# HarborYuan/PolyphonicFormer

Hardware: AMD Instinct MI355X
Metric: frames/sec kernel-update+mask fwd, 1024x2048 N=153 S=3 (higher is better)
Workload: dtype bf16 (feature planes as given; query side: updator half hi/lo bf16, attention / FFN / towers one fp16 plane; one fp16 plane of dynamic kernels, fp16 logits)

## Files before the change

### polyphonicformer_amd/csrc/ph_query.hip

```cpp
#include <stdlib.h>

#include "ph_common.h"

template <int E> __device__ __forceinline__ uint32_t q_f2e(float x) {
    if constexpr (E == PH_E_F16) return f2h(__builtin_amdgcn_fmed3f(x, -65504.f, 65504.f));
    else return f2bf(x);
}

constexpr int LDA = 264;
constexpr float LN_EPS = 1e-5f;

constexpr int NW = 8;
constexpr int CT = 2;
constexpr int WCOLS = CT * 16;
constexpr int NTHREADS = NW * 64;

template <int NRT> struct Tile { f32x4_t v[NRT][CT]; };


struct QArgs {
    const float* partial; const uint32_t* bits; const float* k_in; const float* q_in;
    const uint16_t* wb; const float* wf;
    float* obj; float* dobj; float* cls; uint16_t* kern; float* kbias;
    uint16_t* Qp; uint16_t* Kp; uint16_t* Vt; float* o1;
    ph_stage_layout lay;
    int nsplit, B, N, Npad, cls_sigmoid, kern_f16;
    int64_t HWp;
    const int32_t* pcount;
};

__device__ __forceinline__ int q_lane(int lane) {
    asm volatile("" : "+v"(lane));
    return lane;
}

template <int NRT> __device__ __forceinline__ void tile_zero(f32x4_t (&a)[NRT][CT]) {
#pragma unroll
    for (int rt = 0; rt < NRT; ++rt)
#pragma unroll
        for (int ct = 0; ct < CT; ++ct) a[rt][ct] = f32x4_t{0.f, 0.f, 0.f, 0.f};
}

template <int NRT>
__device__ __forceinline__ void tile_add_bias(Tile<NRT>& t, const float* __restrict__ bias, int wave, int lane) {
#pragma unroll
    for (int ct = 0; ct < CT; ++ct) {
        const float bv = bias[wave * WCOLS + ct * 16 + (lane & 15)];
#pragma unroll
        for (int rt = 0; rt < NRT; ++rt)
#pragma unroll
            for (int r = 0; r < 4; ++r) t.v[rt][ct][r] += bv;
    }
}

template <int PA, int NRT, int E = PH_E_BF16>
__device__ __forceinline__ void tile_to_lds(const Tile<NRT>& t, uint16_t* dst, int plane, int wave, int lane) {
    lane = q_lane(lane);
    const int i = lane & 15, g = lane >> 4;
#pragma unroll
    for (int rt = 0; rt < NRT; ++rt)
#pragma unroll
        for (int ct = 0; ct < CT; ++ct)
#pragma unroll
            for (int r = 0; r < 4; ++r) {
                const int off = (rt * 16 + g * 4 + r) * LDA + wave * WCOLS + ct * 16 + i;
                if (PA == 1) dst[off] = (uint16_t)q_f2e<E>(t.v[rt][ct][r]);
                else {
                    uint32_t hi, lo;
                    f2bf_split(t.v[rt][ct][r], hi, lo);
                    dst[off] = (uint16_t)hi;
                    dst[off + plane] = (uint16_t)lo;
                }
            }
}

template <int NRT, int NT>
__device__ __forceinline__ void ln_row_totals(float* red, int pass, int tid) {
    constexpr int ROWS = NRT * 16;
    for (int idx = tid; idx < NT * ROWS; idx += NTHREADS) {
        float* p = red + ((pass * NT + idx / ROWS) * NW) * ROWS + idx % ROWS;
        float tot = 0.f;
#pragma unroll
        for (int w = 0; w < NW; ++w) tot += p[w * ROWS];
        p[0] = tot;
    }
    __syncthreads();
}
template <int NRT, int NT>
__device__ __forceinline__ void ln_tiles(Tile<NRT> (&t)[NT], const float* const (&gam)[NT], const float* const (&bet)[NT],
                                         float* red, int wave, int lane) {
    constexpr int ROWS = NRT * 16;
    lane = q_lane(lane);
    const int i = lane & 15, g = lane >> 4;
    float mean[NT][NRT][4];
#pragma unroll
    for (int n = 0; n < NT; ++n)
#pragma unroll
        for (int rt = 0; rt < NRT; ++rt)
#pragma unroll
            for (int r = 0; r < 4; ++r) {
                float s = 0.f;
#pragma unroll
                for (int ct = 0; ct < CT; ++ct) s += t[n].v[rt][ct][r];
                s = wave_group16_sum(s);
                if (i == 0) red[((0 * NT + n) * NW + wave) * ROWS + rt * 16 + g * 4 + r] = s;
            }
    __syncthreads();
    ln_row_totals<NRT, NT>(red, 0, wave * 64 + lane);
#pragma unroll
    for (int n = 0; n < NT; ++n)
#pragma unroll
        for (int rt = 0; rt < NRT; ++rt) {
            __builtin_amdgcn_sched_barrier(0);
            asm volatile("" ::: "memory");
#pragma unroll
            for (int r = 0; r < 4; ++r) {
                const float tot = red[(0 * NT + n) * NW * ROWS + rt * 16 + g * 4 + r];
                mean[n][rt][r] = tot * (1.f / 256.f);
                float s = 0.f;
#pragma unroll
                for (int ct = 0; ct < CT; ++ct) {
                    const float d = t[n].v[rt][ct][r] - mean[n][rt][r];
                    t[n].v[rt][ct][r] = d;
                    s += d * d;
                }
                s = wave_group16_sum(s);
                if (i == 0) red[((1 * NT + n) * NW + wave) * ROWS + rt * 16 + g * 4 + r] = s;
            }
#pragma unroll
            for (int ct = 0; ct < CT; ++ct) asm volatile("" : "+v"(t[n].v[rt][ct]));
        }
    __syncthreads();
    ln_row_totals<NRT, NT>(red, 1, wave * 64 + lane);
#pragma unroll
    for (int n = 0; n < NT; ++n) {
        float gm[CT], bt[CT];
#pragma unroll
        for (int ct = 0; ct < CT; ++ct) {
            gm[ct] = gam[n][wave * WCOLS + ct * 16 + i];
            bt[ct] = bet[n][wave * WCOLS + ct * 16 + i];
        }
#pragma unroll
        for (int rt = 0; rt < NRT; ++rt) {
            __builtin_amdgcn_sched_barrier(0);
            asm volatile("" ::: "memory");
#pragma unroll
            for (int r = 0; r < 4; ++r) {
                const float tot = red[(1 * NT + n) * NW * ROWS + rt * 16 + g * 4 + r];
                const float var = tot * (1.f / 256.f);
                const float rstd = fast_rsqrt(var + LN_EPS);
#pragma unroll
                for (int ct = 0; ct < CT; ++ct) t[n].v[rt][ct][r] = t[n].v[rt][ct][r] * rstd * gm[ct] + bt[ct];
            }
#pragma unroll
            for (int ct = 0; ct < CT; ++ct) asm volatile("" : "+v"(t[n].v[rt][ct]));
        }
    }
}

template <int PA, int NRT, int PART, bool QF16 = false>
__device__ __forceinline__ void store_qkv(const Tile<NRT>& T, const QArgs& a, const float* bias, int64_t qk_base,
                                          int64_t qk_plane, int64_t vt_base, int wave, int lane) {
    lane = q_lane(lane);
    const int i = lane & 15, g = lane >> 4;
#pragma unroll
    for (int ct = 0; ct < CT; ++ct) {
        const int col = wave * WCOLS + ct * 16 + i;
        const float bv = bias[col];
#pragma unroll
        for (int rt = 0; rt < NRT; ++rt) {
            uint32_t hi[4], lo[4];
#pragma unroll
            for (int r = 0; r < 4; ++r) {
                float v = T.v[rt][ct][r] + bv;
                if (PART == 0) v *= 0.17677669529663687f;
                if (QF16) { hi[r] = q_f2e<PH_E_F16>(v); lo[r] = 0; }
                else if (PA == 2) f2bf_split(v, hi[r], lo[r]);
                else hi[r] = f2bf(v);
            }
            if (PART < 2) {
                uint16_t* dst = (PART == 0 ? a.Qp : a.Kp) + qk_base + (rt * 16 + g * 4) * 256 + col;
#pragma unroll
                for (int r = 0; r < 4; ++r) {
                    dst[r * 256] = (uint16_t)hi[r];
                    if (PA == 2 && !QF16) dst[qk_plane + r * 256] = (uint16_t)lo[r];
                }
            } else {
                uint16_t* dst = a.Vt + vt_base + (int64_t)col * a.Npad + rt * 16 + g * 4;
                *(uint2*)dst = make_uint2(pack2(hi[0], hi[1]), pack2(hi[2], hi[3]));
                if (PA == 2 && !QF16) *(uint2*)(dst + qk_plane) = make_uint2(pack2(lo[0], lo[1]), pack2(lo[2], lo[3]));
            }
        }
    }
}

constexpr int LDPT = 40;

struct WRef2 { const uint16_t* W; int ct0, ks_total, wks0; };
template <int PA> constexpr int kch() { return PA == 1 ? 4 : 2; }
template <int NCT> struct WStreamF { uint4 f[2][4][NCT]; };
template <int PA, int NCT> using WStream = WStreamF<NCT>;

template <int PA, int NCT>
__device__ __forceinline__ void w_chunk_load(uint4 (&d)[4][NCT], const WRef2& r, int kc, int64_t w_plane, int lane) {
#pragma unroll
    for (int p = 0; p < PA; ++p)
#pragma unroll
        for (int k = 0; k < kch<PA>(); ++k)
#pragma unroll
            for (int ct = 0; ct < NCT; ++ct)
                d[p * kch<PA>() + k][ct] = *(const uint4*)(r.W + p * w_plane + ((int64_t)(r.ct0 + ct) * r.ks_total + r.wks0 + kc * kch<PA>() + k) * 512 + lane * 8);
}
template <int PA, int NCT>
__device__ __forceinline__ void w_prime(WStream<PA, NCT>& ws, const WRef2& r, int64_t w_plane, int lane) {
    w_chunk_load<PA, NCT>(ws.f[0], r, 0, w_plane, lane);
}
struct NoNext { __device__ __forceinline__ void operator()() const {} };

template <int PA, int NRT, int NCT, int NKS, int E = PH_E_BF16, typename Next>
__device__ __forceinline__ void gemm_stream(f32x4_t (&acc)[NRT][NCT], const uint16_t* A, int lda, int a_plane, WStream<PA, NCT>& ws,
                                            const WRef2& r, int64_t w_plane, int lane, Next next) {
    constexpr int KCH = kch<PA>(), NCH = NKS / KCH;
    static_assert(NKS % KCH == 0 && NCH % 2 == 0, "a call is an even number of chunks");
    constexpr int RG = PA == 2 ? 1 : (NRT < 2 ? NRT : 2);
    const int i = lane & 15, g = lane >> 4;
    __builtin_amdgcn_sched_barrier(0);
#pragma unroll
    for (int kc = 0; kc < NCH; ++kc) {
        if (kc + 1 < NCH) w_chunk_load<PA, NCT>(ws.f[(kc + 1) & 1], r, kc + 1, w_plane, lane);
        else next();
        __builtin_amdgcn_sched_barrier(0);
#pragma unroll
        for (int k = 0; k < KCH; ++k)
#pragma unroll
            for (int rt0 = 0; rt0 < NRT; rt0 += RG) {
                uint4 a[PA][RG];
#pragma unroll
                for (int p = 0; p < PA; ++p)
#pragma unroll
                    for (int rr = 0; rr < RG && rt0 + rr < NRT; ++rr)
                        a[p][rr] = *(const uint4*)(A + p * a_plane + ((rt0 + rr) * 16 + i) * lda + (kc * KCH + k) * 32 + g * 8);
#pragma unroll
                for (int ct = 0; ct < NCT; ++ct)
#pragma unroll
                    for (int rr = 0; rr < RG && rt0 + rr < NRT; ++rr) {
                        f32x4_t& c = acc[rt0 + rr][ct];
                        c = mfma16e<E>(a[0][rr], ws.f[kc & 1][k][ct], c);
                        if (PA == 2) {
                            c = mfma16(a[0][rr], ws.f[kc & 1][(PA - 1) * KCH + k][ct], c);
                            c = mfma16(a[PA - 1][rr], ws.f[kc & 1][k][ct], c);
                        }
                    }
            }
        __builtin_amdgcn_sched_barrier(0);
    }
}

template <int PA, int NRT, int NCT, int E = PH_E_BF16>
__device__ __forceinline__ void frag_to_lds(const f32x4_t (&t)[NRT][NCT], uint16_t* dst, int ld, int plane, int col0, int lane) {
    lane = q_lane(lane);
    const int i = lane & 15, g = lane >> 4;
#pragma unroll
    for (int rt = 0; rt < NRT; ++rt)
#pragma unroll
        for (int ct = 0; ct < NCT; ++ct)
#pragma unroll
            for (int r = 0; r < 4; ++r) {
                const int off = (rt * 16 + g * 4 + r) * ld + col0 + ct * 16 + i;
                if (PA == 1) dst[off] = (uint16_t)q_f2e<E>(t[rt][ct][r]);
                else {
                    uint32_t hi, lo;
                    f2bf_split(t[rt][ct][r], hi, lo);
                    dst[off] = (uint16_t)hi;
                    dst[off + plane] = (uint16_t)lo;
                }
            }
}

struct QArgs2 {
    QArgs q;
    unsigned long long* tl;
    float* pi;
    int br0, nbr;
};

#define PH_TL(k)                                                                                             \
    do {                                                                                                     \
        if (aa.tl && blockIdx.x == 0 && blockIdx.y == 0 && blockIdx.z == 0 && threadIdx.x == 0)              \
            aa.tl[(k)] = __builtin_amdgcn_s_memrealtime();                                                   \
    } while (0)

template <int PA, int NRT, bool QF16 = false>
__global__ __launch_bounds__(NTHREADS) void k_query_pre2(const QArgs2 aa) {
    const QArgs& a = aa.q;
    constexpr int ROWS = NRT * 16;
    constexpr int PLANE = ROWS * LDA;
    extern __shared__ __attribute__((aligned(16))) unsigned char smem[];
    uint16_t* act = (uint16_t*)smem;
    float* red = (float*)(act + PA * PLANE);
    float* cnt = red + 2 * 2 * NW * ROWS;

    const int tid = threadIdx.x, lane = tid & 63;
    const int wave = __builtin_amdgcn_readfirstlane(tid >> 6);
    const int i = lane & 15, g = lane >> 4;
    const int row0 = blockIdx.x * ROWS, br = blockIdx.y + aa.br0, b = blockIdx.z;
    const int N = a.N, Npad = a.Npad;
    const uint16_t* wb = a.wb;
    const int64_t wpl = a.lay.wb_plane_elems;
    const float* wf = a.wf;
    const int64_t* WO = a.lay.w[br];
    const int64_t* VO = a.lay.v[br];
    float* pi = aa.pi + ((((int64_t)b * 2 + br) * Npad + row0) * 2) * 256;

    WStream<PA, CT> ws;
    const WRef2 c_dyn_o{wb + WO[PH_W_DYN], 16 + wave * CT, 8, 0}, c_dyn_i{wb + WO[PH_W_DYN], wave * CT, 8, 0};
    const WRef2 c_inp_i{wb + WO[PH_W_INP], wave * CT, 8, 0}, c_inp_o{wb + WO[PH_W_INP], 16 + wave * CT, 8, 0};
    const WRef2 c_ug{wb + WO[PH_W_UG], wave * CT, 8, 0}, c_ig{wb + WO[PH_W_IG], wave * CT, 8, 0}, c_fc{wb + WO[PH_W_FC], wave * CT, 8, 0};
    const WRef2 c_q{wb + WO[PH_W_QKV], wave * CT, 8, 0}, c_k{wb + WO[PH_W_QKV], 16 + wave * CT, 8, 0}, c_v{wb + WO[PH_W_QKV], 32 + wave * CT, 8, 0};
    auto prime = [&](const WRef2& r) { return [&, r]() { w_prime<PA, CT>(ws, r, wpl, lane); }; };
    constexpr int PT = QF16 ? 1 : PA;
    constexpr int ET = QF16 ? PH_E_F16 : PH_E_BF16;
    auto primeT = [&](const WRef2& r) { return [&, r]() { w_prime<PT, CT>(ws, r, wpl, lane); }; };
    w_prime<PA, CT>(ws, c_dyn_o, wpl, lane);
    PH_TL(0);

    auto put16 = [&](int rr, int cb, const float (&v)[16]) {
#pragma unroll
        for (int e = 0; e < 16; e += 2) {
            uint32_t h0, l0, h1, l1;
            f2bf_split(v[e], h0, l0); f2bf_split(v[e + 1], h1, l1);
            *(uint32_t*)(act + rr * LDA + cb + e) = pack2(h0, h1);
            if (PA == 2) *(uint32_t*)(act + PLANE + rr * LDA + cb + e) = pack2(l0, l1);
        }
    };

    {
        const int r = tid >> 5, cb = (tid & 31) * 8;
        for (int rr = r; rr < ROWS; rr += NTHREADS / 32) {
            const int row = row0 + rr;
            float u[8];
#pragma unroll
            for (int e = 0; e < 8; ++e) u[e] = 0.f;
            int c = 0;
            if (row < Npad) {
                if (a.pcount) {
                    for (int s0 = tid & 31; s0 < a.nsplit; s0 += 32) c += a.pcount[((int64_t)b * a.nsplit + s0) * Npad + row];
                } else {
                    const uint4* bw = (const uint4*)(a.bits + ((int64_t)b * Npad + row) * (a.HWp / 32));
                    const int nq = (int)(a.HWp / 128);
                    for (int w0 = tid & 31; w0 < nq; w0 += 256) {
                        uint4 q[8];
#pragma unroll
                        for (int j = 0; j < 8; ++j) q[j] = w0 + 32 * j < nq ? bw[w0 + 32 * j] : make_uint4(0, 0, 0, 0);
#pragma unroll
                        for (int j = 0; j < 8; ++j) c += __popc(q[j].x) + __popc(q[j].y) + __popc(q[j].z) + __popc(q[j].w);
                    }
                }
                constexpr int TRIP = NRT == 1 ? 16 : 8;
                for (int s0 = 0; s0 < a.nsplit; s0 += TRIP) {
                    float4 v[TRIP][2];
#pragma unroll
                    for (int j = 0; j < TRIP; ++j) {
                        const float* p = a.partial + (((int64_t)b * a.nsplit + s0 + j) * Npad + row) * 512 + br * 256 + cb;
#pragma unroll
                        for (int e = 0; e < 2; ++e)
                            v[j][e] = s0 + j < a.nsplit ? *(const float4*)(p + 4 * e) : make_float4(0.f, 0.f, 0.f, 0.f);
                    }
#pragma unroll
                    for (int j = 0; j < TRIP; ++j)
#pragma unroll
                        for (int e = 0; e < 2; ++e) {
                            u[4 * e] += v[j][e].x; u[4 * e + 1] += v[j][e].y; u[4 * e + 2] += v[j][e].z; u[4 * e + 3] += v[j][e].w;
                        }
                }
            }
#pragma unroll
            for (int e = 0; e < 8; e += 2) {
                uint32_t h0, l0, h1, l1;
                f2bf_split(u[e], h0, l0); f2bf_split(u[e + 1], h1, l1);
                *(uint32_t*)(act + rr * LDA + cb + e) = pack2(h0, h1);
                if (PA == 2) *(uint32_t*)(act + PLANE + rr * LDA + cb + e) = pack2(l0, l1);
            }
            float cf = wave_group16_sum((float)c);
            cf += __shfl_xor(cf, 16);
            if ((tid & 31) == 0) cnt[rr] = cf;
        }
    }
    __syncthreads();

    PH_TL(1);
    const float* vc = wf + VO[PH_V_DYN_CNT];
    const float* bd = wf + VO[PH_V_DYN_B];
    {
        Tile<NRT> Po[1];
        tile_zero(Po[0].v);
        const int lp = q_lane(lane), i = lp & 15, g = lp >> 4;
        gemm_stream<PA, NRT, CT, 8>(Po[0].v, act, LDA, PLANE, ws, c_dyn_o, wpl, lane, prime(c_dyn_i));
#pragma unroll
        for (int ct = 0; ct < CT; ++ct) {
            const int col = wave * WCOLS + ct * 16 + i;
            const float vc1 = vc[256 + col], bd1 = bd[256 + col];
#pragma unroll
            for (int rt = 0; rt < NRT; ++rt)
#pragma unroll
                for (int r = 0; r < 4; ++r) Po[0].v[rt][ct][r] += cnt[rt * 16 + g * 4 + r] * vc1 + bd1;
        }
        const float* const gm[1] = {wf + VO[PH_V_LN_PO_G]};
        const float* const bt[1] = {wf + VO[PH_V_LN_PO_B]};
        ln_tiles<NRT, 1>(Po, gm, bt, red, wave, lane);
#pragma unroll
        for (int rt = 0; rt < NRT; ++rt)
#pragma unroll
            for (int ct = 0; ct < CT; ++ct)
#pragma unroll
                for (int r = 0; r < 4; ++r)
                    pi[((rt * 16 + g * 4 + r) * 2 + 0) * 256 + wave * WCOLS + ct * 16 + i] = Po[0].v[rt][ct][r];
    }
    Tile<NRT> Pin;
    tile_zero(Pin.v);
    gemm_stream<PA, NRT, CT, 8>(Pin.v, act, LDA, PLANE, ws, c_dyn_i, wpl, lane, prime(c_inp_i));
    {
        const int lp = q_lane(lane), i = lp & 15, g = lp >> 4;
#pragma unroll
        for (int ct = 0; ct < CT; ++ct) {
            const int col = wave * WCOLS + ct * 16 + i;
            const float vc0 = vc[col], bd0 = bd[col];
#pragma unroll
            for (int rt = 0; rt < NRT; ++rt)
#pragma unroll
                for (int r = 0; r < 4; ++r) Pin.v[rt][ct][r] += cnt[rt * 16 + g * 4 + r] * vc0 + bd0;
        }
    }
    __syncthreads();
    PH_TL(2);
    {
        const int r = tid >> 4, cb = (tid & 15) * 16;
        for (int rr = r; rr < ROWS; rr += NTHREADS / 16) {
            const int row = row0 + rr;
            float kv[16];
#pragma unroll
            for (int e = 0; e < 16; ++e) kv[e] = 0.f;
            if (row < N) {
                const float* kp = a.k_in + ((int64_t)b * N + row) * 256 + cb;
#pragma unroll
                for (int e = 0; e < 16; e += 4) {
                    const float4 v = *(const float4*)(kp + e);
                    kv[e] = v.x; kv[e + 1] = v.y; kv[e + 2] = v.z; kv[e + 3] = v.w;
                }
                if (br == 1) {
                    const float* qp = a.q_in + ((int64_t)b * N + row) * 256 + cb;
#pragma unroll
                    for (int e = 0; e < 16; e += 4) {
                        const float4 v = *(const float4*)(qp + e);
                        kv[e] += v.x; kv[e + 1] += v.y; kv[e + 2] += v.z; kv[e + 3] += v.w;
                    }
                }
            }
            put16(rr, cb, kv);
        }
    }
    __syncthreads();
    PH_TL(3);
    const float* bi = wf + VO[PH_V_INP_B];
    {
        Tile<NRT> Iin;
        tile_zero(Iin.v);
        const int lp = q_lane(lane), i = lp & 15, g = lp >> 4;
        gemm_stream<PA, NRT, CT, 8>(Iin.v, act, LDA, PLANE, ws, c_inp_i, wpl, lane, prime(c_inp_o));
#pragma unroll
        for (int ct = 0; ct < CT; ++ct) {
            const float bi0 = bi[wave * WCOLS + ct * 16 + i];
#pragma unroll
            for (int rt = 0; rt < NRT; ++rt)
#pragma unroll
                for (int r = 0; r < 4; ++r) Pin.v[rt][ct][r] = (Iin.v[rt][ct][r] + bi0) * Pin.v[rt][ct][r];
        }
    }
    {
        Tile<NRT> Io[1];
        tile_zero(Io[0].v);
        const int lp = q_lane(lane), i = lp & 15, g = lp >> 4;
        gemm_stream<PA, NRT, CT, 8>(Io[0].v, act, LDA, PLANE, ws, c_inp_o, wpl, lane, prime(c_ug));
#pragma unroll
        for (int ct = 0; ct < CT; ++ct) {
            const float bi1 = bi[256 + wave * WCOLS + ct * 16 + i];
#pragma unroll
            for (int rt = 0; rt < NRT; ++rt)
#pragma unroll
                for (int r = 0; r < 4; ++r) Io[0].v[rt][ct][r] += bi1;
        }
        const float* const gm[1] = {wf + VO[PH_V_LN_IO_G]};
        const float* const bt[1] = {wf + VO[PH_V_LN_IO_B]};
        ln_tiles<NRT, 1>(Io, gm, bt, red, wave, lane);
#pragma unroll
        for (int rt = 0; rt < NRT; ++rt)
#pragma unroll
            for (int ct = 0; ct < CT; ++ct)
#pragma unroll
                for (int r = 0; r < 4; ++r)
                    pi[((rt * 16 + g * 4 + r) * 2 + 1) * 256 + wave * WCOLS + ct * 16 + i] = Io[0].v[rt][ct][r];
    }
    tile_to_lds<PA, NRT>(Pin, act, PLANE, wave, lane);
    __syncthreads();

    PH_TL(4);
    {
        Tile<NRT> Fg;
        auto gate = [&](const WRef2& cur, auto&& next, int b_idx, int g_idx, int be_idx, int which, bool first) {
            Tile<NRT> G[1];
            tile_zero(G[0].v);
            gemm_stream<PA, NRT, CT, 8>(G[0].v, act, LDA, PLANE, ws, cur, wpl, lane, next);
            tile_add_bias(G[0], wf + VO[b_idx], wave, lane);
            const float* const gm[1] = {wf + VO[g_idx]};
            const float* const bt[1] = {wf + VO[be_idx]};
            ln_tiles<NRT, 1>(G, gm, bt, red, wave, lane);
            const int lp = q_lane(lane), i = lp & 15, g = lp >> 4;
#pragma unroll
            for (int rt = 0; rt < NRT; ++rt) {
                float pv[CT][4];
#pragma unroll
                for (int ct = 0; ct < CT; ++ct)
#pragma unroll
                    for (int r = 0; r < 4; ++r) pv[ct][r] = pi[((rt * 16 + g * 4 + r) * 2 + which) * 256 + wave * WCOLS + ct * 16 + i];
#pragma unroll
                for (int ct = 0; ct < CT; ++ct)
#pragma unroll
                    for (int r = 0; r < 4; ++r) {
                        const float t = fast_sigmoid(G[0].v[rt][ct][r]) * pv[ct][r];
                        Fg.v[rt][ct][r] = first ? t : Fg.v[rt][ct][r] + t;
                    }
            }
        };
        gate(c_ug, prime(c_ig), PH_V_UG_B, PH_V_LN_UG_G, PH_V_LN_UG_B, 0, true);
        gate(c_ig, prime(c_fc), PH_V_IG_B, PH_V_LN_IG_G, PH_V_LN_IG_B, 1, false);
        tile_to_lds<PA, NRT>(Fg, act, PLANE, wave, lane);
    }
    __syncthreads();

    PH_TL(5);
    {
        Tile<NRT> O[1];
        tile_zero(O[0].v);
        gemm_stream<PA, NRT, CT, 8>(O[0].v, act, LDA, PLANE, ws, c_fc, wpl, lane, primeT(c_q));
        tile_add_bias(O[0], wf + VO[PH_V_FC_B], wave, lane);
        const float* const gm[1] = {wf + VO[PH_V_LN_FC_G]};
        const float* const bt[1] = {wf + VO[PH_V_LN_FC_B]};
        ln_tiles<NRT, 1>(O, gm, bt, red, wave, lane);
        const int lp = q_lane(lane), i = lp & 15, g = lp >> 4;
        float* o1 = a.o1 + (((int64_t)b * 2 + br) * Npad + row0) * 256;
#pragma unroll
        for (int rt = 0; rt < NRT; ++rt)
#pragma unroll
            for (int ct = 0; ct < CT; ++ct)
#pragma unroll
                for (int r = 0; r < 4; ++r) {
                    const float v = fmaxf(O[0].v[rt][ct][r], 0.f);
                    O[0].v[rt][ct][r] = v;
                    o1[(rt * 16 + g * 4 + r) * 256 + wave * WCOLS + ct * 16 + i] = v;
                }
        tile_to_lds<PT, NRT, ET>(O[0], act, PLANE, wave, lane);
    }
    __syncthreads();

    PH_TL(6);
    const int64_t qk_base = (((int64_t)b * 2 + br) * Npad + row0) * 256;
    const int64_t qk_plane = (int64_t)a.B * 2 * Npad * 256;
    const int64_t vt_base = ((int64_t)b * 2 + br) * 256 * Npad + row0;
    const float* qkv_bias = wf + VO[PH_V_QKV_B];
    {
        Tile<NRT> T;
        tile_zero(T.v);
        gemm_stream<PT, NRT, CT, 8, ET>(T.v, act, LDA, PLANE, ws, c_q, wpl, lane, primeT(c_k));
        store_qkv<PA, NRT, 0, QF16>(T, a, qkv_bias, qk_base, qk_plane, vt_base, wave, lane);
        tile_zero(T.v);
        gemm_stream<PT, NRT, CT, 8, ET>(T.v, act, LDA, PLANE, ws, c_k, wpl, lane, primeT(c_v));
        store_qkv<PA, NRT, 1, QF16>(T, a, qkv_bias + 256, qk_base, qk_plane, vt_base, wave, lane);
        tile_zero(T.v);
        gemm_stream<PT, NRT, CT, 8, ET>(T.v, act, LDA, PLANE, ws, c_v, wpl, lane, NoNext());
        store_qkv<PA, NRT, 2, QF16>(T, a, qkv_bias + 512, qk_base, qk_plane, vt_base, wave, lane);
    }
    PH_TL(7);
}

template <int PA> constexpr int post2_hc() { return PA == 1 ? 256 : 128; }
template <int PA, int NRT> constexpr int post2_nhb() {
    return ((size_t)PA * NRT * 16 * LDA * 2 + 2 * (size_t)PA * NRT * 16 * (post2_hc<PA>() + 8) * 2 + 2 * 2 * NW * NRT * 16 * 4 + NW * PA * 16 * LDPT * 2 <= 150 * 1024) ? 2 : 1;
}

template <int PA, int NRT, int E = PH_E_BF16>
__global__ __launch_bounds__(NTHREADS) void k_query_post2(const QArgs2 aa) {
    const QArgs& a = aa.q;
    constexpr int ROWS = NRT * 16;
    constexpr int PLANE = ROWS * LDA;
    constexpr int HC = post2_hc<PA>(), LDH = HC + 8, CTH = HC / 128;
    constexpr int HPLANE = ROWS * LDH;
    constexpr int NHB = post2_nhb<PA, NRT>();
    extern __shared__ __attribute__((aligned(16))) unsigned char smem[];
    uint16_t* act = (uint16_t*)smem;
    uint16_t* hb = act + PA * PLANE;
    float* red = (float*)(hb + NHB * PA * HPLANE);
    uint16_t* ptile = (uint16_t*)(red + 2 * 2 * NW * ROWS);
    const int Npad = a.Npad, N = a.N;

    const int tid = threadIdx.x, lane = tid & 63;
    const int wave = __builtin_amdgcn_readfirstlane(tid >> 6);
    const int i = lane & 15, g = lane >> 4;
    const int row0 = blockIdx.x * ROWS, br = blockIdx.y + aa.br0, b = blockIdx.z;
    const uint16_t* wb = a.wb;
    const int64_t wpl = a.lay.wb_plane_elems;
    const float* wf = a.wf;
    const int64_t* WO = a.lay.w[br];
    const int64_t* VO = a.lay.v[br];

    const int64_t qk_plane = (int64_t)a.B * 2 * Npad * 256;
    const uint16_t* Qb = a.Qp + (((int64_t)b * 2 + br) * Npad + row0) * 256;
    const uint16_t* Kb = a.Kp + ((int64_t)b * 2 + br) * Npad * 256;
    const uint16_t* Vb = a.Vt + ((int64_t)b * 2 + br) * 256 * Npad;

    WStream<PA, CT> ws;
    WStream<PA, 1> ws1;
    const WRef2 c_out{wb + WO[PH_W_OUT], wave * CT, 8, 0};
    const WRef2 c_h0a{wb + WO[PH_W_H0A], wave * CT, 8, 0}, c_h0b{wb + WO[PH_W_H0B], wave * CT, 8, 0};
    const WRef2 c_kern{wb + WO[PH_W_KERN], wave * CT, 8, 0}, c_kb{wb + WO[PH_W_KERN], 16, 8, 0};
    auto prime = [&](const WRef2& r) { return [&, r]() { w_prime<PA, CT>(ws, r, wpl, lane); }; };
    auto ffn1_ref = [&](int c) { return WRef2{wb + WO[PH_W_FFN1], c * (HC / 16) + wave * CTH, 8, 0}; };
    auto ffn1_prime = [&](int c) {
        if constexpr (CTH == CT) w_prime<PA, CT>(ws, ffn1_ref(c), wpl, lane);
        else w_prime<PA, 1>(ws1, ffn1_ref(c), wpl, lane);
    };
    w_prime<PA, CT>(ws, c_out, wpl, lane);
    PH_TL(8);

    Tile<NRT> At;
    {
        const int h = wave;
        const int nkt = Npad / 16;
        uint16_t* Pt = ptile + wave * (PA * 16 * LDPT);
        uint4 qf[PA][NRT];
#pragma unroll
        for (int p = 0; p < PA; ++p)
#pragma unroll
            for (int rt = 0; rt < NRT; ++rt)
                qf[p][rt] = *(const uint4*)(Qb + p * qk_plane + (rt * 16 + i) * 256 + h * 32 + g * 8);
        float mx[NRT][4], sm[NRT][4];
#pragma unroll
        for (int rt = 0; rt < NRT; ++rt)
#pragma unroll
            for (int r = 0; r < 4; ++r) { mx[rt][r] = -INFINITY; sm[rt][r] = 0.f; }
        auto load_k = [&](uint4 (&kf)[PA], int kt) {
#pragma unroll
            for (int p = 0; p < PA; ++p) kf[p] = *(const uint4*)(Kb + p * qk_plane + (kt * 16 + i) * 256 + h * 32 + g * 8);
        };
        auto score = [&](const uint4 (&kf)[PA], int rt) {
            f32x4_t s = {0.f, 0.f, 0.f, 0.f};
            s = mfma16e<E>(qf[0][rt], kf[0], s);
            if (PA == 2) { s = mfma16(qf[0][rt], kf[PA - 1], s); s = mfma16(qf[PA - 1][rt], kf[0], s); }
            return s;
        };
        for (int kt = 0; kt < nkt; ++kt) {
            uint4 kf[PA];
            load_k(kf, kt);
            const bool valid = kt * 16 + i < N;
#pragma unroll
            for (int rt = 0; rt < NRT; ++rt) {
                const f32x4_t s = score(kf, rt);
#pragma unroll
                for (int r = 0; r < 4; ++r) mx[rt][r] = fmaxf(mx[rt][r], valid ? s[r] : -INFINITY);
            }
        }
#pragma unroll
        for (int rt = 0; rt < NRT; ++rt)
#pragma unroll
            for (int r = 0; r < 4; ++r) mx[rt][r] = wave_group16_max(mx[rt][r]);
        tile_zero(At.v);
        for (int ks = 0; ks < nkt / 2; ++ks) {
            uint4 kf[2][PA], vf[2][PA];
            load_k(kf[0], 2 * ks);
            load_k(kf[1], 2 * ks + 1);
#pragma unroll
            for (int ct = 0; ct < 2; ++ct)
#pragma unroll
                for (int p = 0; p < PA; ++p)
                    vf[ct][p] = *(const uint4*)(Vb + p * qk_plane + (int64_t)(h * 32 + ct * 16 + i) * Npad + ks * 32 + g * 8);
#pragma unroll
            for (int rt = 0; rt < NRT; ++rt) {
#pragma unroll
                for (int half = 0; half < 2; ++half) {
                    const f32x4_t s = score(kf[half], rt);
                    const bool valid = (2 * ks + half) * 16 + i < N;
#pragma unroll
                    for (int r = 0; r < 4; ++r) {
                        const float pv = valid ? fast_exp(s[r] - mx[rt][r]) : 0.f;
                        sm[rt][r] += pv;
                        const int off = (g * 4 + r) * LDPT + half * 16 + i;
                        if (PA == 2) {
                            uint32_t hi, lo;
                            f2bf_split(pv, hi, lo);
                            Pt[off] = (uint16_t)hi;
                            Pt[16 * LDPT + off] = (uint16_t)lo;
                        } else Pt[off] = (uint16_t)q_f2e<E>(pv);
                    }
                }
                uint4 pf[PA];
#pragma unroll
                for (int p = 0; p < PA; ++p) pf[p] = *(const uint4*)(Pt + p * 16 * LDPT + i * LDPT + g * 8);
#pragma unroll
                for (int ct = 0; ct < 2; ++ct) {
                    At.v[rt][ct] = mfma16e<E>(pf[0], vf[ct][0], At.v[rt][ct]);
                    if (PA == 2) {
                        At.v[rt][ct] = mfma16(pf[0], vf[ct][PA - 1], At.v[rt][ct]);
                        At.v[rt][ct] = mfma16(pf[PA - 1], vf[ct][0], At.v[rt][ct]);
                    }
                }
            }
        }
#pragma unroll
        for (int rt = 0; rt < NRT; ++rt)
#pragma unroll
            for (int r = 0; r < 4; ++r) {
                const float inv = fast_rcp(wave_group16_sum(sm[rt][r]));
#pragma unroll
                for (int ct = 0; ct < 2; ++ct) At.v[rt][ct][r] *= inv;
            }
    }
    tile_to_lds<PA, NRT, E>(At, act, PLANE, wave, lane);
    __syncthreads();

    PH_TL(9);
    Tile<NRT> O2[1];
    tile_zero(O2[0].v);
    gemm_stream<PA, NRT, CT, 8, E>(O2[0].v, act, LDA, PLANE, ws, c_out, wpl, lane, [&]() { ffn1_prime(0); });
    tile_add_bias(O2[0], wf + VO[PH_V_OUT_B], wave, lane);
    {
        const float* o1 = a.o1 + (((int64_t)b * 2 + br) * Npad + row0) * 256;
#pragma unroll
        for (int rt = 0; rt < NRT; ++rt)
#pragma unroll
            for (int ct = 0; ct < CT; ++ct)
#pragma unroll
                for (int r = 0; r < 4; ++r) O2[0].v[rt][ct][r] += o1[(rt * 16 + g * 4 + r) * 256 + wave * WCOLS + ct * 16 + i];
        const float* const gm[1] = {wf + VO[PH_V_LN_ATT_G]};
        const float* const bt[1] = {wf + VO[PH_V_LN_ATT_B]};
        ln_tiles<NRT, 1>(O2, gm, bt, red, wave, lane);
    }
    tile_to_lds<PA, NRT, E>(O2[0], act, PLANE, wave, lane);
    float* park = aa.pi + ((((int64_t)b * 2 + br) * Npad + row0) * 2) * 256;
#pragma unroll
    for (int rt = 0; rt < NRT; ++rt)
#pragma unroll
        for (int ct = 0; ct < CT; ++ct)
#pragma unroll
            for (int r = 0; r < 4; ++r) park[(rt * 16 + g * 4 + r) * 512 + wave * WCOLS + ct * 16 + i] = O2[0].v[rt][ct][r];
    __syncthreads();

    PH_TL(10);
    Tile<NRT> O3[1];
    tile_zero(O3[0].v);
    {
        const int nchunk = a.lay.ffn_dim / HC;
        const int ffn_ks = a.lay.ffn_dim / 32;
        for (int c = 0; c < nchunk; ++c) {
            uint16_t* hc = hb + (NHB == 2 ? (c & 1) : 0) * PA * HPLANE;
            const WRef2 w2{wb + WO[PH_W_FFN2], wave * CT, ffn_ks, c * (HC / 32)};
            f32x4_t Hc[NRT][CTH];
#pragma unroll
            for (int rt = 0; rt < NRT; ++rt)
#pragma unroll
                for (int ct = 0; ct < CTH; ++ct) Hc[rt][ct] = f32x4_t{0.f, 0.f, 0.f, 0.f};
            if constexpr (CTH == CT) gemm_stream<PA, NRT, CT, 8, E>(Hc, act, LDA, PLANE, ws, ffn1_ref(c), wpl, lane, prime(w2));
            else gemm_stream<PA, NRT, 1, 8, E>(Hc, act, LDA, PLANE, ws1, ffn1_ref(c), wpl, lane, prime(w2));
#pragma unroll
            for (int ct = 0; ct < CTH; ++ct) {
                const float bv = (wf + VO[PH_V_FFN1_B])[c * HC + (wave * CTH + ct) * 16 + i];
#pragma unroll
                for (int rt = 0; rt < NRT; ++rt)
#pragma unroll
                    for (int r = 0; r < 4; ++r) Hc[rt][ct][r] = fmaxf(Hc[rt][ct][r] + bv, 0.f);
            }
            if (NHB == 1 && c > 0) __syncthreads();
            frag_to_lds<PA, NRT, CTH, E>(Hc, hc, LDH, HPLANE, wave * CTH * 16, lane);
            __syncthreads();
            gemm_stream<PA, NRT, CT, HC / 32, E>(O3[0].v, hc, LDH, HPLANE, ws, w2, wpl, lane, [&]() {
                if (c + 1 < nchunk) ffn1_prime(c + 1);
                else w_prime<PA, CT>(ws, br == 0 ? c_h0b : c_h0a, wpl, lane);
            });
        }
    }
    PH_TL(11);
    tile_add_bias(O3[0], wf + VO[PH_V_FFN2_B], wave, lane);
#pragma unroll
    for (int rt = 0; rt < NRT; ++rt)
#pragma unroll
        for (int ct = 0; ct < CT; ++ct)
#pragma unroll
            for (int r = 0; r < 4; ++r) O3[0].v[rt][ct][r] += park[(rt * 16 + g * 4 + r) * 512 + wave * WCOLS + ct * 16 + i];
    {
        const float* const gm[1] = {wf + VO[PH_V_LN_FFN_G]};
        const float* const bt[1] = {wf + VO[PH_V_LN_FFN_B]};
        ln_tiles<NRT, 1>(O3, gm, bt, red, wave, lane);
    }
    {
        float* out = (br == 0 ? a.obj : a.dobj) + ((int64_t)b * N + row0) * 256;
#pragma unroll
        for (int rt = 0; rt < NRT; ++rt)
#pragma unroll
            for (int ct = 0; ct < CT; ++ct)
#pragma unroll
                for (int r = 0; r < 4; ++r) {
                    const int rr = rt * 16 + g * 4 + r;
                    if (row0 + rr < N) out[rr * 256 + wave * WCOLS + ct * 16 + i] = O3[0].v[rt][ct][r];
                }
    }
    tile_to_lds<PA, NRT, E>(O3[0], act, PLANE, wave, lane);
    __syncthreads();

    PH_TL(12);
    Tile<NRT> Hm[1];
    if (br == 0) {
        tile_zero(Hm[0].v);
        gemm_stream<PA, NRT, CT, 8, E>(Hm[0].v, act, LDA, PLANE, ws, c_h0b, wpl, lane, prime(c_h0a));
        {
            const float* const gm[1] = {wf + VO[PH_V_LN_H0B_G]};
            const float* const bt[1] = {wf + VO[PH_V_LN_H0B_B]};
            ln_tiles<NRT, 1>(Hm, gm, bt, red, wave, lane);
        }
        Tile<NRT> Hd[1];
        tile_zero(Hd[0].v);
        const int L = a.lay.num_classes, nct = (L + 15) / 16;
        auto cls_ref = [&](int ct) { return WRef2{wb + WO[PH_W_CLS], ct, 8, 0}; };
        gemm_stream<PA, NRT, CT, 8, E>(Hd[0].v, act, LDA, PLANE, ws, c_h0a, wpl, lane, [&]() {
            w_prime<PA, CT>(ws, c_kern, wpl, lane);
            if (wave < nct) w_prime<PA, 1>(ws1, cls_ref(wave), wpl, lane);
        });
        {
            const float* const gm[1] = {wf + VO[PH_V_LN_H0A_G]};
            const float* const bt[1] = {wf + VO[PH_V_LN_H0A_B]};
            ln_tiles<NRT, 1>(Hd, gm, bt, red, wave, lane);
        }
#pragma unroll
        for (int rt = 0; rt < NRT; ++rt)
#pragma unroll
            for (int ct = 0; ct < CT; ++ct)
#pragma unroll
                for (int r = 0; r < 4; ++r) {
                    Hd[0].v[rt][ct][r] = fmaxf(Hd[0].v[rt][ct][r], 0.f);
                    Hm[0].v[rt][ct][r] = fmaxf(Hm[0].v[rt][ct][r], 0.f);
                }
        tile_to_lds<PA, NRT, E>(Hd[0], act, PLANE, wave, lane);
        __syncthreads();
        const float* bc = wf + VO[PH_V_CLS_B];
        for (int ct = wave; ct < nct; ct += NW) {
            f32x4_t acc[NRT][1];
#pragma unroll
            for (int rt = 0; rt < NRT; ++rt) acc[rt][0] = f32x4_t{0.f, 0.f, 0.f, 0.f};
            gemm_stream<PA, NRT, 1, 8, E>(acc, act, LDA, PLANE, ws1, cls_ref(ct), wpl, lane, [&]() {
                if (ct + NW < nct) w_prime<PA, 1>(ws1, cls_ref(ct + NW), wpl, lane);
            });
            const int col = ct * 16 + i;
            if (col < L) {
                const float bv = bc[col];
#pragma unroll
                for (int rt = 0; rt < NRT; ++rt)
#pragma unroll
                    for (int r = 0; r < 4; ++r) {
                        const int row = row0 + rt * 16 + g * 4 + r;
                        if (row < N) {
                            const float z = acc[rt][0][r] + bv;
                            a.cls[((int64_t)b * N + row) * L + col] = a.cls_sigmoid ? fast_sigmoid(z) : z;
                        }
                    }
            }
        }
        __syncthreads();
    } else {
        tile_zero(Hm[0].v);
        gemm_stream<PA, NRT, CT, 8, E>(Hm[0].v, act, LDA, PLANE, ws, c_h0a, wpl, lane, prime(c_kern));
        const float* const gm[1] = {wf + VO[PH_V_LN_H0A_G]};
        const float* const bt[1] = {wf + VO[PH_V_LN_H0A_B]};
        ln_tiles<NRT, 1>(Hm, gm, bt, red, wave, lane);
    }
    tile_to_lds<PA, NRT, E>(Hm[0], act, PLANE, wave, lane);
    __syncthreads();
    {
        Tile<NRT> Kt;
        tile_zero(Kt.v);
        gemm_stream<PA, NRT, CT, 8, E>(Kt.v, act, LDA, PLANE, ws, c_kern, wpl, lane, [&]() {
            if (wave == 0) w_prime<PA, 1>(ws1, c_kb, wpl, lane);
        });
        const float* bk = wf + VO[PH_V_KERN_B];
        const int64_t kplane = (int64_t)2 * a.B * Npad * 256;
        uint16_t* kd = a.kern + (((int64_t)br * a.B + b) * Npad + row0) * 256;
#pragma unroll
        for (int ct = 0; ct < CT; ++ct) {
            const int col = wave * WCOLS + ct * 16 + i;
            const float bv = bk[col];
#pragma unroll
            for (int rt = 0; rt < NRT; ++rt)
#pragma unroll
                for (int r = 0; r < 4; ++r) {
                    const int off = (rt * 16 + g * 4 + r) * 256 + col;
                    if (a.kern_f16) {
                        kd[off] = (uint16_t)q_f2e<PH_E_F16>(Kt.v[rt][ct][r] + bv);
                    } else {
                        uint32_t hi, lo;
                        f2bf_split(Kt.v[rt][ct][r] + bv, hi, lo);
                        kd[off] = (uint16_t)hi;
                        if (PA == 2) kd[kplane + off] = (uint16_t)lo;
                    }
                }
        }
        if (wave == 0) {
            f32x4_t acc[NRT][1];
#pragma unroll
            for (int rt = 0; rt < NRT; ++rt) acc[rt][0] = f32x4_t{0.f, 0.f, 0.f, 0.f};
            gemm_stream<PA, NRT, 1, 8, E>(acc, act, LDA, PLANE, ws1, c_kb, wpl, lane, NoNext());
            if (i == 0) {
                const float bv = bk[256];
#pragma unroll
                for (int rt = 0; rt < NRT; ++rt)
#pragma unroll
                    for (int r = 0; r < 4; ++r)
                        a.kbias[((int64_t)br * a.B + b) * Npad + row0 + rt * 16 + g * 4 + r] = acc[rt][0][r] + bv;
            }
        }
    }
    PH_TL(13);
}

static size_t q_ws_bytes(int B, int Npad, int PA) {
    return (size_t)PA * 3 * B * 2 * Npad * 256 * sizeof(uint16_t) + (size_t)3 * B * 2 * Npad * 256 * sizeof(float);
}

extern "C" size_t ph_query_workspace_updator_offset(int B, int N, int prec) {
    return (size_t)((prec == PH_PREC_SPLIT || prec == PH_PREC_QHYBRID) ? 2 : 1) * 3 * B * 2 * ph_n_padded(N) * 256 * sizeof(uint16_t);
}

extern "C" size_t ph_query_workspace_bytes(int B, int N, int prec) {
    return q_ws_bytes(B, ph_n_padded(N), (prec == PH_PREC_SPLIT || prec == PH_PREC_QHYBRID) ? 2 : 1);
}

template <int PA, int NRT, bool HY = false>
static void launch_query2(const QArgs2& a, int phases, hipStream_t s) {
    constexpr int ROWS = NRT * 16;
    if constexpr (HY) {
        static_assert(PA == 2, "hybrid = split pre kernel");
        const size_t red = 2 * 2 * NW * ROWS * sizeof(float);
        const size_t lds_pre = (size_t)2 * ROWS * LDA * 2 + red + ROWS * sizeof(float);
        const size_t lds_post = (size_t)ROWS * LDA * 2 + (size_t)post2_nhb<1, NRT>() * ROWS * (post2_hc<1>() + 8) * 2 + red + (size_t)NW * 16 * LDPT * 2;
        static const bool once = [] {
            (void)hipFuncSetAttribute((const void*)k_query_pre2<2, NRT, true>, hipFuncAttributeMaxDynamicSharedMemorySize, 160 * 1024);
            (void)hipFuncSetAttribute((const void*)k_query_post2<1, NRT, PH_E_F16>, hipFuncAttributeMaxDynamicSharedMemorySize, 160 * 1024);
            return true;
        }();
        (void)once;
        const dim3 grid(a.q.Npad / ROWS, a.nbr, a.q.B);
        if (phases & 1) hipLaunchKernelGGL((k_query_pre2<2, NRT, true>), grid, dim3(NTHREADS), lds_pre, s, a);
        if (phases & 2) hipLaunchKernelGGL((k_query_post2<1, NRT, PH_E_F16>), grid, dim3(NTHREADS), lds_post, s, a);
        return;
    }
    const size_t red = 2 * 2 * NW * ROWS * sizeof(float);
    const size_t lds_pre = (size_t)PA * ROWS * LDA * 2 + red + ROWS * sizeof(float);
    const size_t lds_post = (size_t)PA * ROWS * LDA * 2 + (size_t)post2_nhb<PA, NRT>() * PA * ROWS * (post2_hc<PA>() + 8) * 2 + red +
                            (size_t)NW * PA * 16 * LDPT * 2;
    static const bool once = [] {
        (void)hipFuncSetAttribute((const void*)k_query_pre2<PA, NRT>, hipFuncAttributeMaxDynamicSharedMemorySize, 160 * 1024);
        (void)hipFuncSetAttribute((const void*)k_query_post2<PA, NRT>, hipFuncAttributeMaxDynamicSharedMemorySize, 160 * 1024);
        return true;
    }();
    (void)once;
    const dim3 grid(a.q.Npad / ROWS, a.nbr, a.q.B);
    if (phases & 1) hipLaunchKernelGGL((k_query_pre2<PA, NRT>), grid, dim3(NTHREADS), lds_pre, s, a);
    if (phases & 2) hipLaunchKernelGGL((k_query_post2<PA, NRT>), grid, dim3(NTHREADS), lds_post, s, a);
}

static int query_run(const PhQueryKnobs& kn, const float* partial, int nsplit, const uint32_t* bits, const int32_t* pcount, const float* k_in,
                     const float* q_in, const uint16_t* wb, const float* wf, const ph_stage_layout* layout, float* obj, float* dobj,
                     float* cls, int cls_sigmoid, uint16_t* kern, float* kbias, void* workspace,
                     size_t workspace_bytes, int B, int N, int64_t HW, int prec, int kern_format, int phases,
                     void* stream) {
    PH_CHECK_ARG((phases & ~(PH_QUERY_BOTH | PH_QUERY_WIDE | PH_QUERY_MASK_ONLY | PH_QUERY_DEPTH_ONLY)) == 0 && (phases & PH_QUERY_BOTH) != 0 &&
                     (phases & (PH_QUERY_MASK_ONLY | PH_QUERY_DEPTH_ONLY)) != (PH_QUERY_MASK_ONLY | PH_QUERY_DEPTH_ONLY),
                 "phases must be PH_QUERY_PRE | PH_QUERY_POST [| PH_QUERY_WIDE] [| PH_QUERY_MASK_ONLY or PH_QUERY_DEPTH_ONLY]");
    PH_CHECK_ARG(partial && bits && k_in && q_in && wb && wf && layout && obj && dobj && cls && kern && kbias && workspace,
                 "null pointer");
    PH_CHECK_ARG(B > 0 && N > 0 && N <= 256 && HW > 0 && nsplit >= 1, "bad size");
    PH_CHECK_ARG(prec == PH_PREC_BF16 || prec == PH_PREC_SPLIT || prec == PH_PREC_QHYBRID, "prec must be PH_PREC_BF16, PH_PREC_SPLIT or PH_PREC_QHYBRID");
    PH_CHECK_ARG(kern_format == PH_KERN_BF16_PLANES || kern_format == PH_KERN_F16, "bad kern_format");
    PH_CHECK_ARG(prec != PH_PREC_QHYBRID || kern_format == PH_KERN_F16, "PH_PREC_QHYBRID emits the dynamic kernels as one fp16 plane (PH_KERN_F16)");
    PH_CHECK_ARG(layout->ffn_dim > 0 && layout->ffn_dim % 256 == 0, "ffn_dim must be a multiple of 256");
    PH_CHECK_ARG(layout->num_classes > 0 && layout->num_classes <= 1024, "bad num_classes");
    const bool hybrid = prec == PH_PREC_QHYBRID;
    const int PA = (prec == PH_PREC_SPLIT || hybrid) ? 2 : 1, Npad = ph_n_padded(N);
    const bool wide = (phases & PH_QUERY_WIDE) != 0;
    const int br0 = (phases & PH_QUERY_DEPTH_ONLY) ? 1 : 0, nbr = (phases & (PH_QUERY_MASK_ONLY | PH_QUERY_DEPTH_ONLY)) ? 1 : 2;
    phases &= PH_QUERY_BOTH;
    if (workspace_bytes < q_ws_bytes(B, Npad, PA)) {
        ph_set_error("ph_query_stage: workspace too small (%zu < %zu)", workspace_bytes, q_ws_bytes(B, Npad, PA));
        return PH_EWORKSPACE;
    }
    QArgs a;
    a.partial = partial; a.bits = bits; a.pcount = pcount; a.k_in = k_in; a.q_in = q_in; a.wb = wb; a.wf = wf;
    a.obj = obj; a.dobj = dobj; a.cls = cls; a.kern = kern; a.kbias = kbias;
    const size_t pl = (size_t)PA * B * 2 * Npad * 256;
    a.Qp = (uint16_t*)workspace; a.Kp = a.Qp + pl; a.Vt = a.Kp + pl; a.o1 = (float*)(a.Vt + pl);
    a.lay = *layout; a.cls_sigmoid = cls_sigmoid; a.kern_f16 = kern_format == PH_KERN_F16; a.nsplit = nsplit; a.B = B; a.N = N; a.Npad = Npad; a.HWp = ph_hw_padded(HW);
    hipStream_t s = (hipStream_t)stream;
    QArgs2 a2;
    a2.q = a;
    unsigned long long* tl = kn.timeline;
    a2.tl = tl;
    a2.pi = a.o1 + (size_t)B * 2 * Npad * 256;
    a2.br0 = br0; a2.nbr = nbr;
    const int t = Npad / 16;
    int nrt = 1;
    if (wide) {
        nrt = t % 5 == 0 ? 5 : (t % 4 == 0 ? 4 : (t % 3 == 0 ? 3 : (t % 2 == 0 ? 2 : 1)));
    } else {
        int smallest = 1;
        for (int c = 5; c >= 2; --c) {
            if (t % c) continue;
            smallest = c;
            if (nrt == 1 && (int64_t)B * 2 * (t / c) >= 200) nrt = c;
        }
        if (nrt == 1) nrt = smallest;
    }
    if (kn.nrt > 0) { nrt = kn.nrt; while (t % nrt) --nrt; }
#define PH_Q2(P, R) launch_query2<P, R>(a2, phases, s)
#define PH_QH(R) launch_query2<2, R, true>(a2, phases, s)
    if (hybrid) { switch (nrt) { case 5: PH_QH(5); break; case 4: PH_QH(4); break; case 3: PH_QH(3); break; case 2: PH_QH(2); break; default: PH_QH(1); } }
    else if (PA == 1) { switch (nrt) { case 5: PH_Q2(1, 5); break; case 4: PH_Q2(1, 4); break; case 3: PH_Q2(1, 3); break; case 2: PH_Q2(1, 2); break; default: PH_Q2(1, 1); } }
    else { switch (nrt) { case 5: PH_Q2(2, 5); break; case 4: PH_Q2(2, 4); break; case 3: PH_Q2(2, 3); break; case 2: PH_Q2(2, 2); break; default: PH_Q2(2, 1); } }
#undef PH_Q2
#undef PH_QH
    if (tl) {
        unsigned long long h[16];
        (void)hipStreamSynchronize(s);
        (void)hipMemcpy(h, tl, sizeof(h), hipMemcpyDeviceToHost);
        fprintf(stderr, "query timeline (100 MHz ticks, x10 ns):");
        for (int k = 1; k < 14; ++k) fprintf(stderr, " %s%lld", k == 8 ? "| " : "", (long long)(h[k] - h[k - 1]));
        fprintf(stderr, "\n");
    }
    PH_CHECK_LAUNCH();
    return PH_OK;
}

static PhQueryKnobs query_switches() {
    PhQueryKnobs k;
    k.nrt = ph_switch(PH_SWITCH_QUERY_NRT);
    if (ph_switch(PH_SWITCH_QUERY_TIMELINE)) {
        static unsigned long long* const tl = [] {
            unsigned long long* p = nullptr;
            if (hipMalloc((void**)&p, 16 * sizeof(unsigned long long)) == hipSuccess) (void)hipMemset(p, 0, 128);
            return p;
        }();
        k.timeline = tl;
    }
    return k;
}

extern "C" int ph_query_stage(const float* partial, int nsplit, const uint32_t* bits, const float* k_in, const float* q_in,
                              const uint16_t* wb, const float* wf, const ph_stage_layout* layout, float* obj, float* dobj,
                              float* cls, int cls_sigmoid, uint16_t* kern, float* kbias, void* workspace,
                              size_t workspace_bytes, int B, int N, int64_t HW, int prec, int kern_format, int phases,
                              void* stream) {
    return query_run(query_switches(), partial, nsplit, bits, nullptr, k_in, q_in, wb, wf, layout, obj, dobj, cls, cls_sigmoid, kern, kbias, workspace,
                     workspace_bytes, B, N, HW, prec, kern_format, phases, stream);
}

extern "C" int ph_query_stage_counts(const float* partial, int nsplit, const uint32_t* bits, const int32_t* pcount, const float* k_in,
                                     const float* q_in, const uint16_t* wb, const float* wf, const ph_stage_layout* layout,
                                     float* obj, float* dobj, float* cls, int cls_sigmoid, uint16_t* kern, float* kbias,
                                     void* workspace, size_t workspace_bytes, int B, int N, int64_t HW, int prec, int kern_format,
                                     int phases, void* stream) {
    if (!pcount) { ph_set_error("ph_query_stage_counts: null pcount"); return PH_EINVAL; }
    return query_run(query_switches(), partial, nsplit, bits, pcount, k_in, q_in, wb, wf, layout, obj, dobj, cls, cls_sigmoid, kern, kbias,
                     workspace, workspace_bytes, B, N, HW, prec, kern_format, phases, stream);
}

int ph_query_stage_counts_k(const PhQueryKnobs& kn, const float* partial, int nsplit, const uint32_t* bits, const int32_t* pcount,
                            const float* k_in, const float* q_in, const uint16_t* wb, const float* wf, const ph_stage_layout* layout,
                            float* obj, float* dobj, float* cls, int cls_sigmoid, uint16_t* kern, float* kbias, void* workspace,
                            size_t workspace_bytes, int B, int N, int64_t HW, int prec, int kern_format, int phases, void* stream) {
    if (!pcount) { ph_set_error("ph_query_stage_counts: null pcount"); return PH_EINVAL; }
    return query_run(kn, partial, nsplit, bits, pcount, k_in, q_in, wb, wf, layout, obj, dobj, cls, cls_sigmoid, kern, kbias, workspace,
                     workspace_bytes, B, N, HW, prec, kern_format, phases, stream);
}
```

Before: 18150.

## Swap MFMA operands so query-side accumulators hold rows per lane, vectorize epilogues

Adds a RowLane fragment layout in which gemm_stream swaps the MFMA A/B operands. Each lane then holds four consecutive columns of one row instead of four rows of one column. LayerNorm row reductions, bias adds, LDS writebacks and the global stores of Q/K, dynamic kernels and class logits can then use 4-wide vector accesses and cheaper two-step shuffles, in place of scalar 16-bit stores and 16-lane group sums. V^T keeps the old column layout. This touches many epilogues at once, and the new vector paths rely on alignment assumptions, with a scalar fallback kept for cls.

Result: no change. 18060 (-0.5%).

```diff
diff --git a/polyphonicformer_amd/csrc/ph_query.hip b/polyphonicformer_amd/csrc/ph_query.hip
--- a/polyphonicformer_amd/csrc/ph_query.hip
+++ b/polyphonicformer_amd/csrc/ph_query.hip
@@ -15,7 +15,10 @@
 constexpr int WCOLS = CT * 16;
 constexpr int NTHREADS = NW * 64;
 
-template <int NRT> struct Tile { f32x4_t v[NRT][CT]; };
+struct RowLane {};
+struct ColLane {};
+template <int NRT, int NCT, typename LAY = RowLane> struct Frag { f32x4_t v[NRT][NCT]; };
+template <int NRT, typename LAY = RowLane> using Tile = Frag<NRT, CT, LAY>;
 
 
 struct QArgs {
@@ -34,36 +37,68 @@
     return lane;
 }
 
-template <int NRT> __device__ __forceinline__ void tile_zero(f32x4_t (&a)[NRT][CT]) {
+__device__ __forceinline__ int q_uniform(int x) {
+    asm volatile("" : "+s"(x));
+    return x;
+}
+
+template <int NRT, int NCT, typename LAY> __device__ __forceinline__ void tile_zero(Frag<NRT, NCT, LAY>& t) {
 #pragma unroll
     for (int rt = 0; rt < NRT; ++rt)
 #pragma unroll
-        for (int ct = 0; ct < CT; ++ct) a[rt][ct] = f32x4_t{0.f, 0.f, 0.f, 0.f};
-}
-
-template <int NRT>
-__device__ __forceinline__ void tile_add_bias(Tile<NRT>& t, const float* __restrict__ bias, int wave, int lane) {
-#pragma unroll
-    for (int ct = 0; ct < CT; ++ct) {
-        const float bv = bias[wave * WCOLS + ct * 16 + (lane & 15)];
-#pragma unroll
-        for (int rt = 0; rt < NRT; ++rt)
-#pragma unroll
-            for (int r = 0; r < 4; ++r) t.v[rt][ct][r] += bv;
-    }
-}
-
-template <int PA, int NRT, int E = PH_E_BF16>
-__device__ __forceinline__ void tile_to_lds(const Tile<NRT>& t, uint16_t* dst, int plane, int wave, int lane) {
+        for (int ct = 0; ct < NCT; ++ct) t.v[rt][ct] = f32x4_t{0.f, 0.f, 0.f, 0.f};
+}
+
+__device__ __forceinline__ f32x4_t ld4(const float* p) { return *(const f32x4_t*)p; }
+__device__ __forceinline__ void st4(float* p, f32x4_t v) { *(f32x4_t*)p = v; }
+
+template <int PA, int E>
+__device__ __forceinline__ void pack4(f32x4_t v, uint2& hi, uint2& lo) {
+    uint32_t h[4], l[4];
+#pragma unroll
+    for (int r = 0; r < 4; ++r) {
+        if (PA == 1) { h[r] = q_f2e<E>(v[r]); l[r] = 0; }
+        else f2bf_split(v[r], h[r], l[r]);
+    }
+    hi = make_uint2(pack2(h[0], h[1]), pack2(h[2], h[3]));
+    lo = make_uint2(pack2(l[0], l[1]), pack2(l[2], l[3]));
+}
+
+template <int NRT, int NCT>
+__device__ __forceinline__ void tile_add_bias(Frag<NRT, NCT, RowLane>& t, const float* __restrict__ bias, int lane) {
+#pragma unroll
+    for (int ct = 0; ct < NCT; ++ct) {
+        const f32x4_t bv = ld4(bias + ct * 16 + (lane >> 4) * 4);
+#pragma unroll
+        for (int rt = 0; rt < NRT; ++rt) t.v[rt][ct] += bv;
+    }
+}
+
+template <int PA, int E = PH_E_BF16, int NRT, int NCT>
+__device__ __forceinline__ void frag_to_lds(const Frag<NRT, NCT, RowLane>& t, uint16_t* dst, int ld, int plane, int col0, int lane) {
+    lane = q_lane(lane);
+    uint16_t* d = dst + (lane & 15) * ld + col0 + (lane >> 4) * 4;
+#pragma unroll
+    for (int rt = 0; rt < NRT; ++rt)
+#pragma unroll
+        for (int ct = 0; ct < NCT; ++ct) {
+            uint2 hi, lo;
+            pack4<PA, E>(t.v[rt][ct], hi, lo);
+            *(uint2*)(d + rt * 16 * ld + ct * 16) = hi;
+            if (PA == 2) *(uint2*)(d + plane + rt * 16 * ld + ct * 16) = lo;
+        }
+}
+template <int PA, int E = PH_E_BF16, int NRT, int NCT>
+__device__ __forceinline__ void frag_to_lds(const Frag<NRT, NCT, ColLane>& t, uint16_t* dst, int ld, int plane, int col0, int lane) {
     lane = q_lane(lane);
     const int i = lane & 15, g = lane >> 4;
 #pragma unroll
     for (int rt = 0; rt < NRT; ++rt)
 #pragma unroll
-        for (int ct = 0; ct < CT; ++ct)
+        for (int ct = 0; ct < NCT; ++ct)
 #pragma unroll
             for (int r = 0; r < 4; ++r) {
-                const int off = (rt * 16 + g * 4 + r) * LDA + wave * WCOLS + ct * 16 + i;
+                const int off = (rt * 16 + g * 4 + r) * ld + col0 + ct * 16 + i;
                 if (PA == 1) dst[off] = (uint16_t)q_f2e<E>(t.v[rt][ct][r]);
                 else {
                     uint32_t hi, lo;
@@ -73,6 +108,10 @@
                 }
             }
 }
+template <int PA, int NRT, int E = PH_E_BF16, typename LAY>
+__device__ __forceinline__ void tile_to_lds(const Tile<NRT, LAY>& t, uint16_t* dst, int plane, int wave, int lane) {
+    frag_to_lds<PA, E>(t, dst, LDA, plane, wave * WCOLS, lane);
+}
 
 template <int NRT, int NT>
 __device__ __forceinline__ void ln_row_totals(float* red, int pass, int tid) {
@@ -86,81 +125,97 @@
     }
     __syncthreads();
 }
+__device__ __forceinline__ float row4_sum(float s) {
+    s += __shfl_xor(s, 16);
+    s += __shfl_xor(s, 32);
+    return s;
+}
 template <int NRT, int NT>
-__device__ __forceinline__ void ln_tiles(Tile<NRT> (&t)[NT], const float* const (&gam)[NT], const float* const (&bet)[NT],
+__device__ __forceinline__ void ln_tiles(Tile<NRT, RowLane> (&t)[NT], const float* const (&gam)[NT], const float* const (&bet)[NT],
                                          float* red, int wave, int lane) {
     constexpr int ROWS = NRT * 16;
+    const int i = lane & 15, g = lane >> 4;
+#pragma unroll
+    for (int n = 0; n < NT; ++n)
+#pragma unroll
+        for (int rt = 0; rt < NRT; ++rt) {
+            float p[4];
+#pragma unroll
+            for (int r = 0; r < 4; ++r) {
+                p[r] = 0.f;
+#pragma unroll
+                for (int ct = 0; ct < CT; ++ct) p[r] += t[n].v[rt][ct][r];
+            }
+            const float s = row4_sum((p[0] + p[1]) + (p[2] + p[3]));
+            if (g == 0) red[((0 * NT + n) * NW + wave) * ROWS + rt * 16 + i] = s;
+        }
+    __syncthreads();
+    ln_row_totals<NRT, NT>(red, 0, wave * 64 + lane);
+#pragma unroll
+    for (int n = 0; n < NT; ++n)
+#pragma unroll
+        for (int rt = 0; rt < NRT; ++rt) {
+            const float mean = red[(0 * NT + n) * NW * ROWS + rt * 16 + i] * (1.f / 256.f);
+            float p[4];
+#pragma unroll
+            for (int r = 0; r < 4; ++r) {
+                p[r] = 0.f;
+#pragma unroll
+                for (int ct = 0; ct < CT; ++ct) {
+                    const float d = t[n].v[rt][ct][r] - mean;
+                    t[n].v[rt][ct][r] = d;
+                    p[r] += d * d;
+                }
+            }
+            const float s = row4_sum((p[0] + p[1]) + (p[2] + p[3]));
+            if (g == 0) red[((1 * NT + n) * NW + wave) * ROWS + rt * 16 + i] = s;
+        }
+    __syncthreads();
+    ln_row_totals<NRT, NT>(red, 1, wave * 64 + lane);
+#pragma unroll
+    for (int n = 0; n < NT; ++n) {
+        f32x4_t gm[CT], bt[CT];
+#pragma unroll
+        for (int ct = 0; ct < CT; ++ct) {
+            gm[ct] = ld4(gam[n] + wave * WCOLS + ct * 16 + g * 4);
+            bt[ct] = ld4(bet[n] + wave * WCOLS + ct * 16 + g * 4);
+        }
+#pragma unroll
+        for (int rt = 0; rt < NRT; ++rt) {
+            const float var = red[(1 * NT + n) * NW * ROWS + rt * 16 + i] * (1.f / 256.f);
+            const float rstd = fast_rsqrt(var + LN_EPS);
+#pragma unroll
+            for (int ct = 0; ct < CT; ++ct) t[n].v[rt][ct] = t[n].v[rt][ct] * rstd * gm[ct] + bt[ct];
+        }
+    }
+}
+
+template <int PA, int NRT, int PART, bool QF16 = false>
+__device__ __forceinline__ void store_qkv(const Tile<NRT, RowLane>& T, const QArgs& a, const float* bias, int64_t qk_base,
+                                          int64_t qk_plane, int64_t vt_base, int wave, int lane) {
+    static_assert(PART < 2, "V^T is stored from a ColLane tile");
+    constexpr int PS = QF16 ? 1 : PA, ES = QF16 ? PH_E_F16 : PH_E_BF16;
     lane = q_lane(lane);
-    const int i = lane & 15, g = lane >> 4;
-    float mean[NT][NRT][4];
-#pragma unroll
-    for (int n = 0; n < NT; ++n)
-#pragma unroll
-        for (int rt = 0; rt < NRT; ++rt)
-#pragma unroll
-            for (int r = 0; r < 4; ++r) {
-                float s = 0.f;
-#pragma unroll
-                for (int ct = 0; ct < CT; ++ct) s += t[n].v[rt][ct][r];
-                s = wave_group16_sum(s);
-                if (i == 0) red[((0 * NT + n) * NW + wave) * ROWS + rt * 16 + g * 4 + r] = s;
-            }
-    __syncthreads();
-    ln_row_totals<NRT, NT>(red, 0, wave * 64 + lane);
-#pragma unroll
-    for (int n = 0; n < NT; ++n)
+    const int col0 = wave * WCOLS + (lane >> 4) * 4;
+    uint16_t* dst = (PART == 0 ? a.Qp : a.Kp) + qk_base + (lane & 15) * 256 + col0;
+#pragma unroll
+    for (int ct = 0; ct < CT; ++ct) {
+        const f32x4_t bv = ld4(bias + col0 + ct * 16);
 #pragma unroll
         for (int rt = 0; rt < NRT; ++rt) {
-            __builtin_amdgcn_sched_barrier(0);
-            asm volatile("" ::: "memory");
-#pragma unroll
-            for (int r = 0; r < 4; ++r) {
-                const float tot = red[(0 * NT + n) * NW * ROWS + rt * 16 + g * 4 + r];
-                mean[n][rt][r] = tot * (1.f / 256.f);
-                float s = 0.f;
-#pragma unroll
-                for (int ct = 0; ct < CT; ++ct) {
-                    const float d = t[n].v[rt][ct][r] - mean[n][rt][r];
-                    t[n].v[rt][ct][r] = d;
-                    s += d * d;
-                }
-                s = wave_group16_sum(s);
-                if (i == 0) red[((1 * NT + n) * NW + wave) * ROWS + rt * 16 + g * 4 + r] = s;
-            }
-#pragma unroll
-            for (int ct = 0; ct < CT; ++ct) asm volatile("" : "+v"(t[n].v[rt][ct]));
-        }
-    __syncthreads();
-    ln_row_totals<NRT, NT>(red, 1, wave * 64 + lane);
-#pragma unroll
-    for (int n = 0; n < NT; ++n) {
-        float gm[CT], bt[CT];
-#pragma unroll
-        for (int ct = 0; ct < CT; ++ct) {
-            gm[ct] = gam[n][wave * WCOLS + ct * 16 + i];
-            bt[ct] = bet[n][wave * WCOLS + ct * 16 + i];
-        }
-#pragma unroll
-        for (int rt = 0; rt < NRT; ++rt) {
-            __builtin_amdgcn_sched_barrier(0);
-            asm volatile("" ::: "memory");
-#pragma unroll
-            for (int r = 0; r < 4; ++r) {
-                const float tot = red[(1 * NT + n) * NW * ROWS + rt * 16 + g * 4 + r];
-                const float var = tot * (1.f / 256.f);
-                const float rstd = fast_rsqrt(var + LN_EPS);
-#pragma unroll
-                for (int ct = 0; ct < CT; ++ct) t[n].v[rt][ct][r] = t[n].v[rt][ct][r] * rstd * gm[ct] + bt[ct];
-            }
-#pragma unroll
-            for (int ct = 0; ct < CT; ++ct) asm volatile("" : "+v"(t[n].v[rt][ct]));
-        }
-    }
-}
-
+            f32x4_t v = T.v[rt][ct] + bv;
+            if (PART == 0) v *= 0.17677669529663687f;
+            uint2 hi, lo;
+            pack4<PS, ES>(v, hi, lo);
+            *(uint2*)(dst + rt * 16 * 256 + ct * 16) = hi;
+            if (PS == 2) *(uint2*)(dst + qk_plane + rt * 16 * 256 + ct * 16) = lo;
+        }
+    }
+}
 template <int PA, int NRT, int PART, bool QF16 = false>
-__device__ __forceinline__ void store_qkv(const Tile<NRT>& T, const QArgs& a, const float* bias, int64_t qk_base,
+__device__ __forceinline__ void store_qkv(const Tile<NRT, ColLane>& T, const QArgs& a, const float* bias, int64_t qk_base,
                                           int64_t qk_plane, int64_t vt_base, int wave, int lane) {
+    static_assert(PART == 2, "Q and K are stored from RowLane tiles");
     lane = q_lane(lane);
     const int i = lane & 15, g = lane >> 4;
 #pragma unroll
@@ -172,24 +227,14 @@
             uint32_t hi[4], lo[4];
 #pragma unroll
             for (int r = 0; r < 4; ++r) {
-                float v = T.v[rt][ct][r] + bv;
-                if (PART == 0) v *= 0.17677669529663687f;
+                const float v = T.v[rt][ct][r] + bv;
                 if (QF16) { hi[r] = q_f2e<PH_E_F16>(v); lo[r] = 0; }
                 else if (PA == 2) f2bf_split(v, hi[r], lo[r]);
                 else hi[r] = f2bf(v);
             }
-            if (PART < 2) {
-                uint16_t* dst = (PART == 0 ? a.Qp : a.Kp) + qk_base + (rt * 16 + g * 4) * 256 + col;
-#pragma unroll
-                for (int r = 0; r < 4; ++r) {
-                    dst[r * 256] = (uint16_t)hi[r];
-                    if (PA == 2 && !QF16) dst[qk_plane + r * 256] = (uint16_t)lo[r];
-                }
-            } else {
-                uint16_t* dst = a.Vt + vt_base + (int64_t)col * a.Npad + rt * 16 + g * 4;
-                *(uint2*)dst = make_uint2(pack2(hi[0], hi[1]), pack2(hi[2], hi[3]));
-                if (PA == 2 && !QF16) *(uint2*)(dst + qk_plane) = make_uint2(pack2(lo[0], lo[1]), pack2(lo[2], lo[3]));
-            }
+            uint16_t* dst = a.Vt + vt_base + (int64_t)col * a.Npad + rt * 16 + g * 4;
+            *(uint2*)dst = make_uint2(pack2(hi[0], hi[1]), pack2(hi[2], hi[3]));
+            if (PA == 2 && !QF16) *(uint2*)(dst + qk_plane) = make_uint2(pack2(lo[0], lo[1]), pack2(lo[2], lo[3]));
         }
     }
 }
@@ -217,9 +262,11 @@
 }
 struct NoNext { __device__ __forceinline__ void operator()() const {} };
 
-template <int PA, int NRT, int NCT, int NKS, int E = PH_E_BF16, typename Next>
-__device__ __forceinline__ void gemm_stream(f32x4_t (&acc)[NRT][NCT], const uint16_t* A, int lda, int a_plane, WStream<PA, NCT>& ws,
+template <int PA, int NKS, int E = PH_E_BF16, int NRT, int NCT, typename LAY, typename Next>
+__device__ __forceinline__ void gemm_stream(Frag<NRT, NCT, LAY>& tile, const uint16_t* A, int lda, int a_plane, WStream<PA, NCT>& ws,
                                             const WRef2& r, int64_t w_plane, int lane, Next next) {
+    constexpr bool SW = __is_same(LAY, RowLane);
+    f32x4_t (&acc)[NRT][NCT] = tile.v;
     constexpr int KCH = kch<PA>(), NCH = NKS / KCH;
     static_assert(NKS % KCH == 0 && NCH % 2 == 0, "a call is an even number of chunks");
     constexpr int RG = PA == 2 ? 1 : (NRT < 2 ? NRT : 2);
@@ -245,36 +292,16 @@
 #pragma unroll
                     for (int rr = 0; rr < RG && rt0 + rr < NRT; ++rr) {
                         f32x4_t& c = acc[rt0 + rr][ct];
-                        c = mfma16e<E>(a[0][rr], ws.f[kc & 1][k][ct], c);
+                        const uint4 &whi = ws.f[kc & 1][k][ct], &wlo = ws.f[kc & 1][(PA - 1) * KCH + k][ct];
+                        c = SW ? mfma16e<E>(whi, a[0][rr], c) : mfma16e<E>(a[0][rr], whi, c);
                         if (PA == 2) {
-                            c = mfma16(a[0][rr], ws.f[kc & 1][(PA - 1) * KCH + k][ct], c);
-                            c = mfma16(a[PA - 1][rr], ws.f[kc & 1][k][ct], c);
+                            c = SW ? mfma16(wlo, a[0][rr], c) : mfma16(a[0][rr], wlo, c);
+                            c = SW ? mfma16(whi, a[PA - 1][rr], c) : mfma16(a[PA - 1][rr], whi, c);
                         }
                     }
             }
         __builtin_amdgcn_sched_barrier(0);
     }
-}
-
-template <int PA, int NRT, int NCT, int E = PH_E_BF16>
-__device__ __forceinline__ void frag_to_lds(const f32x4_t (&t)[NRT][NCT], uint16_t* dst, int ld, int plane, int col0, int lane) {
-    lane = q_lane(lane);
-    const int i = lane & 15, g = lane >> 4;
-#pragma unroll
-    for (int rt = 0; rt < NRT; ++rt)
-#pragma unroll
-        for (int ct = 0; ct < NCT; ++ct)
-#pragma unroll
-            for (int r = 0; r < 4; ++r) {
-                const int off = (rt * 16 + g * 4 + r) * ld + col0 + ct * 16 + i;
-                if (PA == 1) dst[off] = (uint16_t)q_f2e<E>(t[rt][ct][r]);
-                else {
-                    uint32_t hi, lo;
-                    f2bf_split(t[rt][ct][r], hi, lo);
-                    dst[off] = (uint16_t)hi;
-                    dst[off + plane] = (uint16_t)lo;
-                }
-            }
 }
 
 struct QArgs2 {
@@ -303,13 +330,13 @@
     const int tid = threadIdx.x, lane = tid & 63;
     const int wave = __builtin_amdgcn_readfirstlane(tid >> 6);
     const int i = lane & 15, g = lane >> 4;
+    const int col0 = wave * WCOLS + g * 4;
     const int row0 = blockIdx.x * ROWS, br = blockIdx.y + aa.br0, b = blockIdx.z;
     const int N = a.N, Npad = a.Npad;
     const uint16_t* wb = a.wb;
     const int64_t wpl = a.lay.wb_plane_elems;
     const float* wf = a.wf;
     const int64_t* WO = a.lay.w[br];
-    const int64_t* VO = a.lay.v[br];
     float* pi = aa.pi + ((((int64_t)b * 2 + br) * Npad + row0) * 2) * 256;
 
     WStream<PA, CT> ws;
@@ -318,6 +345,14 @@
     const WRef2 c_ug{wb + WO[PH_W_UG], wave * CT, 8, 0}, c_ig{wb + WO[PH_W_IG], wave * CT, 8, 0}, c_fc{wb + WO[PH_W_FC], wave * CT, 8, 0};
     const WRef2 c_q{wb + WO[PH_W_QKV], wave * CT, 8, 0}, c_k{wb + WO[PH_W_QKV], 16 + wave * CT, 8, 0}, c_v{wb + WO[PH_W_QKV], 32 + wave * CT, 8, 0};
     auto prime = [&](const WRef2& r) { return [&, r]() { w_prime<PA, CT>(ws, r, wpl, lane); }; };
+    auto park_store = [&](const Tile<NRT>& t, float* dst, int ld) {
+        const int lp = q_lane(lane);
+        float* d = dst + (lp & 15) * ld + wave * WCOLS + (lp >> 4) * 4;
+#pragma unroll
+        for (int rt = 0; rt < NRT; ++rt)
+#pragma unroll
+            for (int ct = 0; ct < CT; ++ct) st4(d + rt * 16 * ld + ct * 16, t.v[rt][ct]);
+    };
     constexpr int PT = QF16 ? 1 : PA;
     constexpr int ET = QF16 ? PH_E_F16 : PH_E_BF16;
     auto primeT = [&](const WRef2& r) { return [&, r]() { w_prime<PT, CT>(ws, r, wpl, lane); }; };
@@ -389,48 +424,33 @@
     __syncthreads();
 
     PH_TL(1);
-    const float* vc = wf + VO[PH_V_DYN_CNT];
-    const float* bd = wf + VO[PH_V_DYN_B];
+    const float* vc = wf + a.lay.v[q_uniform(br)][PH_V_DYN_CNT];
+    const float* bd = wf + a.lay.v[q_uniform(br)][PH_V_DYN_B];
+    auto add_cnt = [&](Tile<NRT>& t, int half) {
+        float c[NRT];
+#pragma unroll
+        for (int rt = 0; rt < NRT; ++rt) c[rt] = cnt[rt * 16 + i];
+#pragma unroll
+        for (int ct = 0; ct < CT; ++ct) {
+            const f32x4_t vcv = ld4(vc + half + col0 + ct * 16), bdv = ld4(bd + half + col0 + ct * 16);
+#pragma unroll
+            for (int rt = 0; rt < NRT; ++rt) t.v[rt][ct] += c[rt] * vcv + bdv;
+        }
+    };
     {
         Tile<NRT> Po[1];
-        tile_zero(Po[0].v);
-        const int lp = q_lane(lane), i = lp & 15, g = lp >> 4;
-        gemm_stream<PA, NRT, CT, 8>(Po[0].v, act, LDA, PLANE, ws, c_dyn_o, wpl, lane, prime(c_dyn_i));
-#pragma unroll
-        for (int ct = 0; ct < CT; ++ct) {
-            const int col = wave * WCOLS + ct * 16 + i;
-            const float vc1 = vc[256 + col], bd1 = bd[256 + col];
-#pragma unroll
-            for (int rt = 0; rt < NRT; ++rt)
-#pragma unroll
-                for (int r = 0; r < 4; ++r) Po[0].v[rt][ct][r] += cnt[rt * 16 + g * 4 + r] * vc1 + bd1;
-        }
-        const float* const gm[1] = {wf + VO[PH_V_LN_PO_G]};
-        const float* const bt[1] = {wf + VO[PH_V_LN_PO_B]};
+        tile_zero(Po[0]);
+        gemm_stream<PA, 8>(Po[0], act, LDA, PLANE, ws, c_dyn_o, wpl, lane, prime(c_dyn_i));
+        add_cnt(Po[0], 256);
+        const float* const gm[1] = {wf + a.lay.v[q_uniform(br)][PH_V_LN_PO_G]};
+        const float* const bt[1] = {wf + a.lay.v[q_uniform(br)][PH_V_LN_PO_B]};
         ln_tiles<NRT, 1>(Po, gm, bt, red, wave, lane);
-#pragma unroll
-        for (int rt = 0; rt < NRT; ++rt)
-#pragma unroll
-            for (int ct = 0; ct < CT; ++ct)
-#pragma unroll
-                for (int r = 0; r < 4; ++r)
-                    pi[((rt * 16 + g * 4 + r) * 2 + 0) * 256 + wave * WCOLS + ct * 16 + i] = Po[0].v[rt][ct][r];
+        park_store(Po[0], pi, 512);
     }
     Tile<NRT> Pin;
-    tile_zero(Pin.v);
-    gemm_stream<PA, NRT, CT, 8>(Pin.v, act, LDA, PLANE, ws, c_dyn_i, wpl, lane, prime(c_inp_i));
-    {
-        const int lp = q_lane(lane), i = lp & 15, g = lp >> 4;
-#pragma unroll
-        for (int ct = 0; ct < CT; ++ct) {
-            const int col = wave * WCOLS + ct * 16 + i;
-            const float vc0 = vc[col], bd0 = bd[col];
-#pragma unroll
-            for (int rt = 0; rt < NRT; ++rt)
-#pragma unroll
-                for (int r = 0; r < 4; ++r) Pin.v[rt][ct][r] += cnt[rt * 16 + g * 4 + r] * vc0 + bd0;
-        }
-    }
+    tile_zero(Pin);
+    gemm_stream<PA, 8>(Pin, act, LDA, PLANE, ws, c_dyn_i, wpl, lane, prime(c_inp_i));
+    add_cnt(Pin, 0);
     __syncthreads();
     PH_TL(2);
     {
@@ -461,44 +481,26 @@
     }
     __syncthreads();
     PH_TL(3);
-    const float* bi = wf + VO[PH_V_INP_B];
+    const float* bi = wf + a.lay.v[q_uniform(br)][PH_V_INP_B];
     {
         Tile<NRT> Iin;
-        tile_zero(Iin.v);
-        const int lp = q_lane(lane), i = lp & 15, g = lp >> 4;
-        gemm_stream<PA, NRT, CT, 8>(Iin.v, act, LDA, PLANE, ws, c_inp_i, wpl, lane, prime(c_inp_o));
-#pragma unroll
-        for (int ct = 0; ct < CT; ++ct) {
-            const float bi0 = bi[wave * WCOLS + ct * 16 + i];
-#pragma unroll
-            for (int rt = 0; rt < NRT; ++rt)
-#pragma unroll
-                for (int r = 0; r < 4; ++r) Pin.v[rt][ct][r] = (Iin.v[rt][ct][r] + bi0) * Pin.v[rt][ct][r];
-        }
+        tile_zero(Iin);
+        gemm_stream<PA, 8>(Iin, act, LDA, PLANE, ws, c_inp_i, wpl, lane, prime(c_inp_o));
+        tile_add_bias(Iin, bi + wave * WCOLS, lane);
+#pragma unroll
+        for (int rt = 0; rt < NRT; ++rt)
+#pragma unroll
+            for (int ct = 0; ct < CT; ++ct) Pin.v[rt][ct] = Iin.v[rt][ct] * Pin.v[rt][ct];
     }
     {
         Tile<NRT> Io[1];
-        tile_zero(Io[0].v);
-        const int lp = q_lane(lane), i = lp & 15, g = lp >> 4;
-        gemm_stream<PA, NRT, CT, 8>(Io[0].v, act, LDA, PLANE, ws, c_inp_o, wpl, lane, prime(c_ug));
-#pragma unroll
-        for (int ct = 0; ct < CT; ++ct) {
-            const float bi1 = bi[256 + wave * WCOLS + ct * 16 + i];
-#pragma unroll
-            for (int rt = 0; rt < NRT; ++rt)
-#pragma unroll
-                for (int r = 0; r < 4; ++r) Io[0].v[rt][ct][r] += bi1;
-        }
-        const float* const gm[1] = {wf + VO[PH_V_LN_IO_G]};
-        const float* const bt[1] = {wf + VO[PH_V_LN_IO_B]};
+        tile_zero(Io[0]);
+        gemm_stream<PA, 8>(Io[0], act, LDA, PLANE, ws, c_inp_o, wpl, lane, prime(c_ug));
+        tile_add_bias(Io[0], bi + 256 + wave * WCOLS, lane);
+        const float* const gm[1] = {wf + a.lay.v[q_uniform(br)][PH_V_LN_IO_G]};
+        const float* const bt[1] = {wf + a.lay.v[q_uniform(br)][PH_V_LN_IO_B]};
         ln_tiles<NRT, 1>(Io, gm, bt, red, wave, lane);
-#pragma unroll
-        for (int rt = 0; rt < NRT; ++rt)
-#pragma unroll
-            for (int ct = 0; ct < CT; ++ct)
-#pragma unroll
-                for (int r = 0; r < 4; ++r)
-                    pi[((rt * 16 + g * 4 + r) * 2 + 1) * 256 + wave * WCOLS + ct * 16 + i] = Io[0].v[rt][ct][r];
+        park_store(Io[0], pi + 256, 512);
     }
     tile_to_lds<PA, NRT>(Pin, act, PLANE, wave, lane);
     __syncthreads();
@@ -508,20 +510,19 @@
         Tile<NRT> Fg;
         auto gate = [&](const WRef2& cur, auto&& next, int b_idx, int g_idx, int be_idx, int which, bool first) {
             Tile<NRT> G[1];
-            tile_zero(G[0].v);
-            gemm_stream<PA, NRT, CT, 8>(G[0].v, act, LDA, PLANE, ws, cur, wpl, lane, next);
-            tile_add_bias(G[0], wf + VO[b_idx], wave, lane);
-            const float* const gm[1] = {wf + VO[g_idx]};
-            const float* const bt[1] = {wf + VO[be_idx]};
+            tile_zero(G[0]);
+            gemm_stream<PA, 8>(G[0], act, LDA, PLANE, ws, cur, wpl, lane, next);
+            tile_add_bias(G[0], wf + a.lay.v[q_uniform(br)][b_idx] + wave * WCOLS, lane);
+            const float* const gm[1] = {wf + a.lay.v[q_uniform(br)][g_idx]};
+            const float* const bt[1] = {wf + a.lay.v[q_uniform(br)][be_idx]};
             ln_tiles<NRT, 1>(G, gm, bt, red, wave, lane);
-            const int lp = q_lane(lane), i = lp & 15, g = lp >> 4;
+            const int lp = q_lane(lane);
+            const float* pr = pi + which * 256 + (lp & 15) * 512 + wave * WCOLS + (lp >> 4) * 4;
 #pragma unroll
             for (int rt = 0; rt < NRT; ++rt) {
-                float pv[CT][4];
-#pragma unroll
-                for (int ct = 0; ct < CT; ++ct)
-#pragma unroll
-                    for (int r = 0; r < 4; ++r) pv[ct][r] = pi[((rt * 16 + g * 4 + r) * 2 + which) * 256 + wave * WCOLS + ct * 16 + i];
+                f32x4_t pv[CT];
+#pragma unroll
+                for (int ct = 0; ct < CT; ++ct) pv[ct] = ld4(pr + rt * 16 * 512 + ct * 16);
 #pragma unroll
                 for (int ct = 0; ct < CT; ++ct)
 #pragma unroll
@@ -540,24 +541,19 @@
     PH_TL(5);
     {
         Tile<NRT> O[1];
-        tile_zero(O[0].v);
-        gemm_stream<PA, NRT, CT, 8>(O[0].v, act, LDA, PLANE, ws, c_fc, wpl, lane, primeT(c_q));
-        tile_add_bias(O[0], wf + VO[PH_V_FC_B], wave, lane);
-        const float* const gm[1] = {wf + VO[PH_V_LN_FC_G]};
-        const float* const bt[1] = {wf + VO[PH_V_LN_FC_B]};
+        tile_zero(O[0]);
+        gemm_stream<PA, 8>(O[0], act, LDA, PLANE, ws, c_fc, wpl, lane, primeT(c_q));
+        tile_add_bias(O[0], wf + a.lay.v[q_uniform(br)][PH_V_FC_B] + wave * WCOLS, lane);
+        const float* const gm[1] = {wf + a.lay.v[q_uniform(br)][PH_V_LN_FC_G]};
+        const float* const bt[1] = {wf + a.lay.v[q_uniform(br)][PH_V_LN_FC_B]};
         ln_tiles<NRT, 1>(O, gm, bt, red, wave, lane);
-        const int lp = q_lane(lane), i = lp & 15, g = lp >> 4;
-        float* o1 = a.o1 + (((int64_t)b * 2 + br) * Npad + row0) * 256;
 #pragma unroll
         for (int rt = 0; rt < NRT; ++rt)
 #pragma unroll
             for (int ct = 0; ct < CT; ++ct)
 #pragma unroll
-                for (int r = 0; r < 4; ++r) {
-                    const float v = fmaxf(O[0].v[rt][ct][r], 0.f);
-                    O[0].v[rt][ct][r] = v;
-                    o1[(rt * 16 + g * 4 + r) * 256 + wave * WCOLS + ct * 16 + i] = v;
-                }
+                for (int r = 0; r < 4; ++r) O[0].v[rt][ct][r] = fmaxf(O[0].v[rt][ct][r], 0.f);
+        park_store(O[0], a.o1 + (((int64_t)b * 2 + br) * Npad + row0) * 256, 256);
         tile_to_lds<PT, NRT, ET>(O[0], act, PLANE, wave, lane);
     }
     __syncthreads();
@@ -566,18 +562,19 @@
     const int64_t qk_base = (((int64_t)b * 2 + br) * Npad + row0) * 256;
     const int64_t qk_plane = (int64_t)a.B * 2 * Npad * 256;
     const int64_t vt_base = ((int64_t)b * 2 + br) * 256 * Npad + row0;
-    const float* qkv_bias = wf + VO[PH_V_QKV_B];
+    const float* qkv_bias = wf + a.lay.v[q_uniform(br)][PH_V_QKV_B];
     {
         Tile<NRT> T;
-        tile_zero(T.v);
-        gemm_stream<PT, NRT, CT, 8, ET>(T.v, act, LDA, PLANE, ws, c_q, wpl, lane, primeT(c_k));
+        tile_zero(T);
+        gemm_stream<PT, 8, ET>(T, act, LDA, PLANE, ws, c_q, wpl, lane, primeT(c_k));
         store_qkv<PA, NRT, 0, QF16>(T, a, qkv_bias, qk_base, qk_plane, vt_base, wave, lane);
-        tile_zero(T.v);
-        gemm_stream<PT, NRT, CT, 8, ET>(T.v, act, LDA, PLANE, ws, c_k, wpl, lane, primeT(c_v));
+        tile_zero(T);
+        gemm_stream<PT, 8, ET>(T, act, LDA, PLANE, ws, c_k, wpl, lane, primeT(c_v));
         store_qkv<PA, NRT, 1, QF16>(T, a, qkv_bias + 256, qk_base, qk_plane, vt_base, wave, lane);
-        tile_zero(T.v);
-        gemm_stream<PT, NRT, CT, 8, ET>(T.v, act, LDA, PLANE, ws, c_v, wpl, lane, NoNext());
-        store_qkv<PA, NRT, 2, QF16>(T, a, qkv_bias + 512, qk_base, qk_plane, vt_base, wave, lane);
+        Tile<NRT, ColLane> V;
+        tile_zero(V);
+        gemm_stream<PT, 8, ET>(V, act, LDA, PLANE, ws, c_v, wpl, lane, NoNext());
+        store_qkv<PA, NRT, 2, QF16>(V, a, qkv_bias + 512, qk_base, qk_plane, vt_base, wave, lane);
     }
     PH_TL(7);
 }
@@ -605,12 +602,12 @@
     const int tid = threadIdx.x, lane = tid & 63;
     const int wave = __builtin_amdgcn_readfirstlane(tid >> 6);
     const int i = lane & 15, g = lane >> 4;
+    const int col0 = wave * WCOLS + g * 4;
     const int row0 = blockIdx.x * ROWS, br = blockIdx.y + aa.br0, b = blockIdx.z;
     const uint16_t* wb = a.wb;
     const int64_t wpl = a.lay.wb_plane_elems;
     const float* wf = a.wf;
     const int64_t* WO = a.lay.w[br];
-    const int64_t* VO = a.lay.v[br];
 
     const int64_t qk_plane = (int64_t)a.B * 2 * Npad * 256;
     const uint16_t* Qb = a.Qp + (((int64_t)b * 2 + br) * Npad + row0) * 256;
@@ -631,7 +628,7 @@
     w_prime<PA, CT>(ws, c_out, wpl, lane);
     PH_TL(8);
 
-    Tile<NRT> At;
+    Tile<NRT, ColLane> At;
     {
         const int h = wave;
         const int nkt = Npad / 16;
@@ -672,7 +669,7 @@
         for (int rt = 0; rt < NRT; ++rt)
 #pragma unroll
             for (int r = 0; r < 4; ++r) mx[rt][r] = wave_group16_max(mx[rt][r]);
-        tile_zero(At.v);
+        tile_zero(At);
         for (int ks = 0; ks < nkt / 2; ++ks) {
             uint4 kf[2][PA], vf[2][PA];
             load_k(kf[0], 2 * ks);
@@ -727,114 +724,100 @@
     __syncthreads();
 
     PH_TL(9);
+    auto add_rows = [&](Tile<NRT>& t, const float* src, int ld) {
+        const int lp = q_lane(lane);
+        const float* p = src + (lp & 15) * ld + wave * WCOLS + (lp >> 4) * 4;
+#pragma unroll
+        for (int rt = 0; rt < NRT; ++rt)
+#pragma unroll
+            for (int ct = 0; ct < CT; ++ct) t.v[rt][ct] += ld4(p + rt * 16 * ld + ct * 16);
+    };
+    auto store_rows = [&](const Tile<NRT>& t, float* dst, int ld, int nrows) {
+        const int lp = q_lane(lane);
+        float* d = dst + (lp & 15) * ld + wave * WCOLS + (lp >> 4) * 4;
+#pragma unroll
+        for (int rt = 0; rt < NRT; ++rt)
+#pragma unroll
+            for (int ct = 0; ct < CT; ++ct)
+                if (rt * 16 + (lp & 15) < nrows) st4(d + rt * 16 * ld + ct * 16, t.v[rt][ct]);
+    };
     Tile<NRT> O2[1];
-    tile_zero(O2[0].v);
-    gemm_stream<PA, NRT, CT, 8, E>(O2[0].v, act, LDA, PLANE, ws, c_out, wpl, lane, [&]() { ffn1_prime(0); });
-    tile_add_bias(O2[0], wf + VO[PH_V_OUT_B], wave, lane);
-    {
-        const float* o1 = a.o1 + (((int64_t)b * 2 + br) * Npad + row0) * 256;
-#pragma unroll
-        for (int rt = 0; rt < NRT; ++rt)
-#pragma unroll
-            for (int ct = 0; ct < CT; ++ct)
-#pragma unroll
-                for (int r = 0; r < 4; ++r) O2[0].v[rt][ct][r] += o1[(rt * 16 + g * 4 + r) * 256 + wave * WCOLS + ct * 16 + i];
-        const float* const gm[1] = {wf + VO[PH_V_LN_ATT_G]};
-        const float* const bt[1] = {wf + VO[PH_V_LN_ATT_B]};
+    tile_zero(O2[0]);
+    gemm_stream<PA, 8, E>(O2[0], act, LDA, PLANE, ws, c_out, wpl, lane, [&]() { ffn1_prime(0); });
+    tile_add_bias(O2[0], wf + a.lay.v[q_uniform(br)][PH_V_OUT_B] + wave * WCOLS, lane);
+    {
+        add_rows(O2[0], a.o1 + (((int64_t)b * 2 + br) * Npad + row0) * 256, 256);
+        const float* const gm[1] = {wf + a.lay.v[q_uniform(br)][PH_V_LN_ATT_G]};
+        const float* const bt[1] = {wf + a.lay.v[q_uniform(br)][PH_V_LN_ATT_B]};
         ln_tiles<NRT, 1>(O2, gm, bt, red, wave, lane);
     }
     tile_to_lds<PA, NRT, E>(O2[0], act, PLANE, wave, lane);
     float* park = aa.pi + ((((int64_t)b * 2 + br) * Npad + row0) * 2) * 256;
-#pragma unroll
-    for (int rt = 0; rt < NRT; ++rt)
-#pragma unroll
-        for (int ct = 0; ct < CT; ++ct)
-#pragma unroll
-            for (int r = 0; r < 4; ++r) park[(rt * 16 + g * 4 + r) * 512 + wave * WCOLS + ct * 16 + i] = O2[0].v[rt][ct][r];
+    store_rows(O2[0], park, 512, ROWS);
     __syncthreads();
 
     PH_TL(10);
     Tile<NRT> O3[1];
-    tile_zero(O3[0].v);
+    tile_zero(O3[0]);
     {
         const int nchunk = a.lay.ffn_dim / HC;
         const int ffn_ks = a.lay.ffn_dim / 32;
         for (int c = 0; c < nchunk; ++c) {
             uint16_t* hc = hb + (NHB == 2 ? (c & 1) : 0) * PA * HPLANE;
             const WRef2 w2{wb + WO[PH_W_FFN2], wave * CT, ffn_ks, c * (HC / 32)};
-            f32x4_t Hc[NRT][CTH];
+            Frag<NRT, CTH> Hc;
+            tile_zero(Hc);
+            if constexpr (CTH == CT) gemm_stream<PA, 8, E>(Hc, act, LDA, PLANE, ws, ffn1_ref(c), wpl, lane, prime(w2));
+            else gemm_stream<PA, 8, E>(Hc, act, LDA, PLANE, ws1, ffn1_ref(c), wpl, lane, prime(w2));
+            tile_add_bias(Hc, wf + a.lay.v[q_uniform(br)][PH_V_FFN1_B] + c * HC + wave * CTH * 16, lane);
 #pragma unroll
             for (int rt = 0; rt < NRT; ++rt)
 #pragma unroll
-                for (int ct = 0; ct < CTH; ++ct) Hc[rt][ct] = f32x4_t{0.f, 0.f, 0.f, 0.f};
-            if constexpr (CTH == CT) gemm_stream<PA, NRT, CT, 8, E>(Hc, act, LDA, PLANE, ws, ffn1_ref(c), wpl, lane, prime(w2));
-            else gemm_stream<PA, NRT, 1, 8, E>(Hc, act, LDA, PLANE, ws1, ffn1_ref(c), wpl, lane, prime(w2));
-#pragma unroll
-            for (int ct = 0; ct < CTH; ++ct) {
-                const float bv = (wf + VO[PH_V_FFN1_B])[c * HC + (wave * CTH + ct) * 16 + i];
-#pragma unroll
-                for (int rt = 0; rt < NRT; ++rt)
-#pragma unroll
-                    for (int r = 0; r < 4; ++r) Hc[rt][ct][r] = fmaxf(Hc[rt][ct][r] + bv, 0.f);
-            }
+                for (int ct = 0; ct < CTH; ++ct)
+#pragma unroll
+                    for (int r = 0; r < 4; ++r) Hc.v[rt][ct][r] = fmaxf(Hc.v[rt][ct][r], 0.f);
             if (NHB == 1 && c > 0) __syncthreads();
-            frag_to_lds<PA, NRT, CTH, E>(Hc, hc, LDH, HPLANE, wave * CTH * 16, lane);
+            frag_to_lds<PA, E>(Hc, hc, LDH, HPLANE, wave * CTH * 16, lane);
             __syncthreads();
-            gemm_stream<PA, NRT, CT, HC / 32, E>(O3[0].v, hc, LDH, HPLANE, ws, w2, wpl, lane, [&]() {
+            gemm_stream<PA, HC / 32, E>(O3[0], hc, LDH, HPLANE, ws, w2, wpl, lane, [&]() {
                 if (c + 1 < nchunk) ffn1_prime(c + 1);
                 else w_prime<PA, CT>(ws, br == 0 ? c_h0b : c_h0a, wpl, lane);
             });
         }
     }
     PH_TL(11);
-    tile_add_bias(O3[0], wf + VO[PH_V_FFN2_B], wave, lane);
-#pragma unroll
-    for (int rt = 0; rt < NRT; ++rt)
-#pragma unroll
-        for (int ct = 0; ct < CT; ++ct)
-#pragma unroll
-            for (int r = 0; r < 4; ++r) O3[0].v[rt][ct][r] += park[(rt * 16 + g * 4 + r) * 512 + wave * WCOLS + ct * 16 + i];
-    {
-        const float* const gm[1] = {wf + VO[PH_V_LN_FFN_G]};
-        const float* const bt[1] = {wf + VO[PH_V_LN_FFN_B]};
+    tile_add_bias(O3[0], wf + a.lay.v[q_uniform(br)][PH_V_FFN2_B] + wave * WCOLS, lane);
+    add_rows(O3[0], park, 512);
+    {
+        const float* const gm[1] = {wf + a.lay.v[q_uniform(br)][PH_V_LN_FFN_G]};
+        const float* const bt[1] = {wf + a.lay.v[q_uniform(br)][PH_V_LN_FFN_B]};
         ln_tiles<NRT, 1>(O3, gm, bt, red, wave, lane);
     }
-    {
-        float* out = (br == 0 ? a.obj : a.dobj) + ((int64_t)b * N + row0) * 256;
-#pragma unroll
-        for (int rt = 0; rt < NRT; ++rt)
-#pragma unroll
-            for (int ct = 0; ct < CT; ++ct)
-#pragma unroll
-                for (int r = 0; r < 4; ++r) {
-                    const int rr = rt * 16 + g * 4 + r;
-                    if (row0 + rr < N) out[rr * 256 + wave * WCOLS + ct * 16 + i] = O3[0].v[rt][ct][r];
-                }
-    }
+    store_rows(O3[0], (br == 0 ? a.obj : a.dobj) + ((int64_t)b * N + row0) * 256, 256, N - row0);
     tile_to_lds<PA, NRT, E>(O3[0], act, PLANE, wave, lane);
     __syncthreads();
 
     PH_TL(12);
     Tile<NRT> Hm[1];
     if (br == 0) {
-        tile_zero(Hm[0].v);
-        gemm_stream<PA, NRT, CT, 8, E>(Hm[0].v, act, LDA, PLANE, ws, c_h0b, wpl, lane, prime(c_h0a));
+        tile_zero(Hm[0]);
+        gemm_stream<PA, 8, E>(Hm[0], act, LDA, PLANE, ws, c_h0b, wpl, lane, prime(c_h0a));
         {
-            const float* const gm[1] = {wf + VO[PH_V_LN_H0B_G]};
-            const float* const bt[1] = {wf + VO[PH_V_LN_H0B_B]};
+            const float* const gm[1] = {wf + a.lay.v[q_uniform(br)][PH_V_LN_H0B_G]};
+            const float* const bt[1] = {wf + a.lay.v[q_uniform(br)][PH_V_LN_H0B_B]};
             ln_tiles<NRT, 1>(Hm, gm, bt, red, wave, lane);
         }
         Tile<NRT> Hd[1];
-        tile_zero(Hd[0].v);
+        tile_zero(Hd[0]);
         const int L = a.lay.num_classes, nct = (L + 15) / 16;
         auto cls_ref = [&](int ct) { return WRef2{wb + WO[PH_W_CLS], ct, 8, 0}; };
-        gemm_stream<PA, NRT, CT, 8, E>(Hd[0].v, act, LDA, PLANE, ws, c_h0a, wpl, lane, [&]() {
+        gemm_stream<PA, 8, E>(Hd[0], act, LDA, PLANE, ws, c_h0a, wpl, lane, [&]() {
             w_prime<PA, CT>(ws, c_kern, wpl, lane);
             if (wave < nct) w_prime<PA, 1>(ws1, cls_ref(wave), wpl, lane);
         });
         {
-            const float* const gm[1] = {wf + VO[PH_V_LN_H0A_G]};
-            const float* const bt[1] = {wf + VO[PH_V_LN_H0A_B]};
+            const float* const gm[1] = {wf + a.lay.v[q_uniform(br)][PH_V_LN_H0A_G]};
+            const float* const bt[1] = {wf + a.lay.v[q_uniform(br)][PH_V_LN_H0A_B]};
             ln_tiles<NRT, 1>(Hd, gm, bt, red, wave, lane);
         }
 #pragma unroll
@@ -848,79 +831,76 @@
                 }
         tile_to_lds<PA, NRT, E>(Hd[0], act, PLANE, wave, lane);
         __syncthreads();
-        const float* bc = wf + VO[PH_V_CLS_B];
+        const float* bc = wf + a.lay.v[q_uniform(br)][PH_V_CLS_B];
+        const bool cls_vec = L % 4 == 0 && ((uintptr_t)a.cls & 15) == 0;
         for (int ct = wave; ct < nct; ct += NW) {
-            f32x4_t acc[NRT][1];
-#pragma unroll
-            for (int rt = 0; rt < NRT; ++rt) acc[rt][0] = f32x4_t{0.f, 0.f, 0.f, 0.f};
-            gemm_stream<PA, NRT, 1, 8, E>(acc, act, LDA, PLANE, ws1, cls_ref(ct), wpl, lane, [&]() {
+            Frag<NRT, 1> acc;
+            tile_zero(acc);
+            gemm_stream<PA, 8, E>(acc, act, LDA, PLANE, ws1, cls_ref(ct), wpl, lane, [&]() {
                 if (ct + NW < nct) w_prime<PA, 1>(ws1, cls_ref(ct + NW), wpl, lane);
             });
-            const int col = ct * 16 + i;
+            const int col = ct * 16 + g * 4;
             if (col < L) {
-                const float bv = bc[col];
-#pragma unroll
-                for (int rt = 0; rt < NRT; ++rt)
-#pragma unroll
-                    for (int r = 0; r < 4; ++r) {
-                        const int row = row0 + rt * 16 + g * 4 + r;
-                        if (row < N) {
-                            const float z = acc[rt][0][r] + bv;
-                            a.cls[((int64_t)b * N + row) * L + col] = a.cls_sigmoid ? fast_sigmoid(z) : z;
+                const f32x4_t bv = ld4(bc + col);
+#pragma unroll
+                for (int rt = 0; rt < NRT; ++rt) {
+                    const int row = row0 + rt * 16 + i;
+                    if (row < N) {
+                        f32x4_t z = acc.v[rt][0] + bv;
+                        if (a.cls_sigmoid) {
+#pragma unroll
+                            for (int r = 0; r < 4; ++r) z[r] = fast_sigmoid(z[r]);
+                        }
+                        float* dst = a.cls + ((int64_t)b * N + row) * L + col;
+                        if (cls_vec) st4(dst, z);
+                        else {
+#pragma unroll
+                            for (int r = 0; r < 4; ++r)
+                                if (col + r < L) dst[r] = z[r];
                         }
                     }
+                }
             }
         }
         __syncthreads();
     } else {
-        tile_zero(Hm[0].v);
-        gemm_stream<PA, NRT, CT, 8, E>(Hm[0].v, act, LDA, PLANE, ws, c_h0a, wpl, lane, prime(c_kern));
-        const float* const gm[1] = {wf + VO[PH_V_LN_H0A_G]};
-        const float* const bt[1] = {wf + VO[PH_V_LN_H0A_B]};
+        tile_zero(Hm[0]);
+        gemm_stream<PA, 8, E>(Hm[0], act, LDA, PLANE, ws, c_h0a, wpl, lane, prime(c_kern));
+        const float* const gm[1] = {wf + a.lay.v[q_uniform(br)][PH_V_LN_H0A_G]};
+        const float* const bt[1] = {wf + a.lay.v[q_uniform(br)][PH_V_LN_H0A_B]};
         ln_tiles<NRT, 1>(Hm, gm, bt, red, wave, lane);
     }
     tile_to_lds<PA, NRT, E>(Hm[0], act, PLANE, wave, lane);
     __syncthreads();
     {
         Tile<NRT> Kt;
-        tile_zero(Kt.v);
-        gemm_stream<PA, NRT, CT, 8, E>(Kt.v, act, LDA, PLANE, ws, c_kern, wpl, lane, [&]() {
+        tile_zero(Kt);
+        gemm_stream<PA, 8, E>(Kt, act, LDA, PLANE, ws, c_kern, wpl, lane, [&]() {
             if (wave == 0) w_prime<PA, 1>(ws1, c_kb, wpl, lane);
         });
-        const float* bk = wf + VO[PH_V_KERN_B];
+        const float* bk = wf + a.lay.v[q_uniform(br)][PH_V_KERN_B];
         const int64_t kplane = (int64_t)2 * a.B * Npad * 256;
-        uint16_t* kd = a.kern + (((int64_t)br * a.B + b) * Npad + row0) * 256;
-#pragma unroll
-        for (int ct = 0; ct < CT; ++ct) {
-            const int col = wave * WCOLS + ct * 16 + i;
-            const float bv = bk[col];
-#pragma unroll
-            for (int rt = 0; rt < NRT; ++rt)
-#pragma unroll
-                for (int r = 0; r < 4; ++r) {
-                    const int off = (rt * 16 + g * 4 + r) * 256 + col;
-                    if (a.kern_f16) {
-                        kd[off] = (uint16_t)q_f2e<PH_E_F16>(Kt.v[rt][ct][r] + bv);
-                    } else {
-                        uint32_t hi, lo;
-                        f2bf_split(Kt.v[rt][ct][r] + bv, hi, lo);
-                        kd[off] = (uint16_t)hi;
-                        if (PA == 2) kd[kplane + off] = (uint16_t)lo;
-                    }
-                }
-        }
+        uint16_t* kd = a.kern + (((int64_t)br * a.B + b) * Npad + row0 + i) * 256 + col0;
+        tile_add_bias(Kt, bk + wave * WCOLS, lane);
+#pragma unroll
+        for (int rt = 0; rt < NRT; ++rt)
+#pragma unroll
+            for (int ct = 0; ct < CT; ++ct) {
+                uint2 hi, lo;
+                if (a.kern_f16) pack4<1, PH_E_F16>(Kt.v[rt][ct], hi, lo);
+                else pack4<2, PH_E_BF16>(Kt.v[rt][ct], hi, lo);
+                *(uint2*)(kd + rt * 16 * 256 + ct * 16) = hi;
+                if (PA == 2 && !a.kern_f16) *(uint2*)(kd + kplane + rt * 16 * 256 + ct * 16) = lo;
+            }
         if (wave == 0) {
-            f32x4_t acc[NRT][1];
-#pragma unroll
-            for (int rt = 0; rt < NRT; ++rt) acc[rt][0] = f32x4_t{0.f, 0.f, 0.f, 0.f};
-            gemm_stream<PA, NRT, 1, 8, E>(acc, act, LDA, PLANE, ws1, c_kb, wpl, lane, NoNext());
-            if (i == 0) {
+            Frag<NRT, 1> acc;
+            tile_zero(acc);
+            gemm_stream<PA, 8, E>(acc, act, LDA, PLANE, ws1, c_kb, wpl, lane, NoNext());
+            if (g == 0) {
                 const float bv = bk[256];
 #pragma unroll
                 for (int rt = 0; rt < NRT; ++rt)
-#pragma unroll
-                    for (int r = 0; r < 4; ++r)
-                        a.kbias[((int64_t)br * a.B + b) * Npad + row0 + rt * 16 + g * 4 + r] = acc[rt][0][r] + bv;
+                    a.kbias[((int64_t)br * a.B + b) * Npad + row0 + rt * 16 + i] = acc.v[rt][0][0] + bv;
             }
         }
     }
```
